# gcorso/disco-diffdock

Measured on AMD Instinct MI355X. Metric: complexes/sec, 20-step 40-sample inference, higher is better.
Workload: dtype f32

## Files before the change

disco_diffdock_amd/_lib.py:

```python
import ctypes as C
import os

_HERE = os.path.dirname(os.path.abspath(__file__))
LIB_PATH = os.environ.get('DDK_LIB') or os.path.join(_HERE, 'libddk.so')


class ddk_config(C.Structure):
    _fields_ = [('ns', C.c_int32), ('nv', C.c_int32), ('num_conv_layers', C.c_int32),
                ('sigma_embed_dim', C.c_int32), ('distance_embed_dim', C.c_int32), ('cross_distance_embed_dim', C.c_int32),
                ('lig_max_radius', C.c_float), ('rec_max_radius', C.c_float), ('cross_max_distance', C.c_float),
                ('center_max_distance', C.c_float), ('dynamic_max_cross', C.c_int32), ('embedding_scale', C.c_float),
                ('scale_by_sigma', C.c_int32), ('no_torsion', C.c_int32), ('batch_norm', C.c_int32),
                ('latent_dim', C.c_int32), ('latent_vocab', C.c_int32), ('latent_droprate', C.c_float),
                ('lm_embedding_dim', C.c_int32),
                ('tr_sigma_min', C.c_float), ('tr_sigma_max', C.c_float), ('rot_sigma_min', C.c_float),
                ('rot_sigma_max', C.c_float), ('tor_sigma_min', C.c_float), ('tor_sigma_max', C.c_float),
                ('device', C.c_int32), ('all_atoms', C.c_int32), ('num_confidence_outputs', C.c_int32),
                ('confidence_no_batchnorm', C.c_int32), ('conv_kernel', C.c_int32), ('deterministic', C.c_int32), ('confidence_mode', C.c_int32)]


class ddk_complex_desc(C.Structure):
    _fields_ = [('n_lig', C.c_int32), ('n_rec', C.c_int32), ('n_bond_edges', C.c_int32), ('n_rot', C.c_int32),
                ('n_rec_edges', C.c_int32), ('rec_feat_dim', C.c_int32),
                ('lig_x', C.c_void_p), ('bond_index', C.c_void_p), ('bond_attr', C.c_void_p), ('edge_mask', C.c_void_p),
                ('mask_rotate', C.c_void_p), ('rec_x', C.c_void_p), ('rec_pos', C.c_void_p), ('rec_edge_index', C.c_void_p)]


class ddk_atoms_desc(C.Structure):
    _fields_ = [('n_atom', C.c_int32), ('n_atom_edges', C.c_int32), ('atom_x', C.c_void_p), ('atom_pos', C.c_void_p),
                ('atom_edge_index', C.c_void_p), ('atom_rec_index', C.c_void_p)]


class ddk_trajectory(C.Structure):
    _fields_ = [('pos', C.c_void_p), ('scores', C.c_void_p), ('perturb', C.c_void_p), ('edge_counts', C.c_void_p)]


class ddk_perturbation(C.Structure):
    _fields_ = [('tr_update', C.c_void_p), ('rot_update', C.c_void_p), ('tor_update', C.c_void_p),
                ('tr_score', C.c_void_p), ('rot_score', C.c_void_p), ('tor_score', C.c_void_p)]


class ddk_match_options(C.Structure):
    _fields_ = [('popsize', C.c_int32), ('maxiter', C.c_int32), ('tol', C.c_float), ('polish_iters', C.c_int32), ('n_islands', C.c_int32),
                ('seed', C.c_uint64), ('stream_id', C.c_uint64)]


_lib = None

SYMBOLS = ['ddk_create', 'ddk_destroy', 'ddk_last_error', 'ddk_version', 'ddk_load_weights', 'ddk_finalize_weights',
           'ddk_set_score_norm_tables', 'ddk_tp_forward', 'ddk_tp_backward', 'ddk_rtp_forward', 'ddk_rtp_backward', 'ddk_rtp_backward_workspace', 'ddk_rconv_forward', 'ddk_rconv_backward', 'ddk_rconv_workspace', 'ddk_rhid_forward', 'ddk_rhid_backward', 'ddk_rhid_workspace', 'ddk_hconv_forward', 'ddk_hconv_backward', 'ddk_hconv_workspace', 'ddk_eemb_forward', 'ddk_eemb_backward', 'ddk_eemb_workspace', 'ddk_eemb_latent_forward', 'ddk_eemb_latent_backward', 'ddk_eemb_latent_workspace', 'ddk_gumbel_softmax_batch', 'ddk_gumbel_softmax_batch_backward', 'ddk_gumbel_pick_samples', 'ddk_rng_latent_keep', 'ddk_node_cross_entropy_batch', 'ddk_node_cross_entropy_batch_backward', 'ddk_rng_decoding_index', 'ddk_seg_sum', 'ddk_conv_forward', 'ddk_complex_create', 'ddk_complex_destroy',
           'ddk_score_forward', 'ddk_se3_update', 'ddk_sample', 'ddk_last_graph_stats', 'ddk_last_node_features',
           'ddk_profile_enable', 'ddk_profile_read', 'ddk_profile_read_forwards', 'ddk_set_latents', 'ddk_set_guidance',
           'ddk_set_keep_receptor_features', 'ddk_randomize_position', 'ddk_complex_set_atoms',
           'ddk_confidence_forward', 'ddk_score_confidence', 'ddk_pose_metrics', 'ddk_build_graph', 'ddk_set_receptive_field_pruning', 'ddk_ar_logits', 'ddk_ar_decode', 'ddk_confidence_status',
           'ddk_sample_trajectory', 'ddk_pose_pairwise_rmsd', 'ddk_pose_cluster',
           'ddk_ligand_automorphisms_workspace', 'ddk_ligand_automorphisms',
           'ddk_receptor_knn_graph_workspace', 'ddk_receptor_knn_graph', 'ddk_radius_graph_workspace', 'ddk_radius_graph',
           'ddk_ligand_transformation_mask_workspace', 'ddk_ligand_transformation_mask',
           'ddk_rng_noise', 'ddk_rng_initial', 'ddk_rng_uniform',
           'ddk_so3_rows', 'ddk_torus_score', 'ddk_rng_perturbation', 'ddk_score_matching_loss',
           'ddk_conformer_match_workspace', 'ddk_conformer_rmsd', 'ddk_conformer_match',
           'ddk_rng_perturbation_batch', 'ddk_rng_forward_times', 'ddk_modify_conformer_batch', 'ddk_randomize_position_batch', 'ddk_score_matching_loss_batch',
           'ddk_score_matching_loss_batch_backward']

DEBUG_SYMBOLS = ['ddk_debug_export', 'ddk_debug_read_edges', 'ddk_debug_conf_counts', 'ddk_debug_conf_table', 'ddk_debug_conf_nodes', 'ddk_debug_conf_edges', 'ddk_debug_kabsch', 'ddk_debug_axis_angle', 'ddk_debug_set_layer0_dedup', 'ddk_debug_read_patch', 'ddk_debug_split3', 'ddk_debug_conv_trace', 'ddk_debug_pool_stats', 'ddk_debug_set_conv_workgroups', 'ddk_debug_set_alloc_limit', 'ddk_debug_cross_mirror']


def lib():
    global _lib
    if _lib is not None:
        return _lib
    if not os.path.exists(LIB_PATH):
        raise RuntimeError(f'{LIB_PATH} not found: build the HIP extension first (python -m disco_diffdock_amd.build). '
                           'disco_diffdock_amd has no CPU fallback.')
    import torch
    L = C.CDLL(LIB_PATH)
    missing = [s for s in SYMBOLS + DEBUG_SYMBOLS if not hasattr(L, s)]
    if missing:
        raise RuntimeError(f'{LIB_PATH} does not export {", ".join(missing)}: it is stale, build the HIP extension again '
                           '(python -m disco_diffdock_amd.build). disco_diffdock_amd has no CPU fallback.')
    vp, i32, i64, f32 = C.c_void_p, C.c_int32, C.c_int64, C.c_float
    L.ddk_create.argtypes = [C.POINTER(ddk_config), C.POINTER(vp)]
    L.ddk_destroy.argtypes = [vp]
    L.ddk_destroy.restype = None
    L.ddk_last_error.argtypes = [vp]
    L.ddk_last_error.restype = C.c_char_p
    L.ddk_version.restype = C.c_char_p
    L.ddk_load_weights.argtypes = [vp, C.c_char_p, vp, C.POINTER(i64), i32]
    L.ddk_finalize_weights.argtypes = [vp]
    L.ddk_set_score_norm_tables.argtypes = [vp, vp, i32, vp, i32]
    L.ddk_tp_forward.argtypes = [vp, i32, vp, vp, vp, i64, vp, vp]
    L.ddk_tp_backward.argtypes = [vp, i32, vp, vp, vp, vp, i64, vp, vp, vp, vp]
    L.ddk_rtp_forward.argtypes = [vp, i32, vp, vp, vp, C.POINTER(i64), i32, vp, vp, i64, vp, vp]
    L.ddk_rtp_backward.argtypes = [vp, i32, vp, vp, vp, C.POINTER(i64), i32, vp, vp, vp, i64, vp, vp, vp, vp, vp, vp, vp]
    L.ddk_rtp_backward_workspace.argtypes = [i32, i64, i32]
    L.ddk_rtp_backward_workspace.restype = i64
    L.ddk_rconv_forward.argtypes = [vp, i32, vp, i64, i64, vp, vp, vp, vp, vp, vp, C.POINTER(i64), i32, vp, vp, i64, vp, vp, vp]
    L.ddk_rconv_backward.argtypes = [vp, i32, vp, i64, i64, vp, vp, vp, vp, vp, vp, vp, vp, C.POINTER(i64), i32, vp, vp, vp, i64, vp, vp, vp, vp, vp, vp, vp]
    L.ddk_rconv_workspace.argtypes = [i32, i64, i32, i64, i64, i32]
    L.ddk_rconv_workspace.restype = i64
    L.ddk_rhid_forward.argtypes = [vp, vp, i64, vp, vp, vp, C.POINTER(i64), i32, vp, vp, f32, C.c_uint64, i64, vp, vp]
    L.ddk_rhid_backward.argtypes = [vp, vp, i64, vp, vp, vp, vp, vp, vp, vp, vp, C.POINTER(i64), i32, vp, vp, f32, i64, vp, vp, vp, vp, vp, vp]
    L.ddk_rhid_workspace.argtypes = [i64, i32, i64]
    L.ddk_rhid_workspace.restype = i64
    L.ddk_hconv_forward.argtypes = [vp, i32, vp, i64, i64, vp, vp, vp, vp, vp, vp, vp, vp, i64, vp, vp, vp]
    L.ddk_hconv_backward.argtypes = [vp, i32, vp, i64, i64, vp, vp, vp, vp, vp, vp, vp, vp, vp, vp, vp, i64, vp, vp, vp, vp, vp, vp]
    L.ddk_hconv_workspace.argtypes = [i32, i64, i64, i64, i32]
    L.ddk_hconv_workspace.restype = i64
    eemb = [vp, vp, i64, vp, i64, vp, vp, vp, i32, vp, i64, vp, f32, f32, i32, vp, vp, vp, vp, f32, C.c_uint64]
    L.ddk_eemb_forward.argtypes = eemb + [i64, vp, vp, vp]
    L.ddk_eemb_backward.argtypes = eemb + [vp, i64, vp, vp, vp, vp, vp, vp]
    L.ddk_eemb_workspace.argtypes = [i64, i32]
    L.ddk_eemb_workspace.restype = i64
    latent = [vp, vp, i32, i32, vp, vp]
    L.ddk_eemb_latent_forward.argtypes = eemb + latent + [i64, vp, vp, vp]
    L.ddk_eemb_latent_backward.argtypes = eemb + latent + [vp, vp, vp, vp, vp, i64, vp, vp, vp, vp, vp, vp, vp, vp, vp]
    L.ddk_eemb_latent_workspace.argtypes = [i64, i32, i32]
    L.ddk_eemb_latent_workspace.restype = i64
    gumbel = [vp, i32, i32, vp, i64, vp, i64, vp, vp, f32]
    L.ddk_gumbel_softmax_batch.argtypes = gumbel + [C.c_uint64, vp, i32, i32, vp, vp, vp, vp, vp]
    L.ddk_gumbel_softmax_batch_backward.argtypes = gumbel + [vp, vp, vp, vp, vp]
    L.ddk_gumbel_pick_samples.argtypes = [vp, i32, i32, vp, i64, vp, i64, f32, C.c_uint64, C.c_uint64, i32, i32, vp, vp, vp, vp]
    L.ddk_rng_latent_keep.argtypes = [vp, C.c_uint64, i32, vp, i32, i32, f32, vp]
    node_ce = [vp, i32, i32, vp, i64, vp, i64, vp, vp, vp, vp, vp, i32]
    L.ddk_node_cross_entropy_batch.argtypes = node_ce + [vp, vp, vp, vp, vp]
    L.ddk_node_cross_entropy_batch_backward.argtypes = node_ce + [vp, vp, vp, vp, vp, vp]
    L.ddk_rng_decoding_index.argtypes = [vp, C.c_uint64, i32, vp, i32, i32, i32, vp]
    L.ddk_seg_sum.argtypes = [vp, vp, vp, vp, vp, i64, i32, vp]
    L.ddk_conv_forward.argtypes = [vp, i32, vp, i64, vp, vp, C.POINTER(i64), vp, vp, vp, vp]
    L.ddk_complex_create.argtypes = [vp, C.POINTER(ddk_complex_desc), i32, C.POINTER(vp)]
    L.ddk_complex_destroy.argtypes = [vp, vp]
    L.ddk_complex_destroy.restype = None
    L.ddk_score_forward.argtypes = [vp, vp, i32, vp, f32, f32, f32, vp, vp, vp, vp]
    L.ddk_se3_update.argtypes = [vp, vp, i32, vp, vp, vp, vp, vp, vp]
    L.ddk_randomize_position.argtypes = [vp, vp, i32, vp, vp, vp, vp, vp, vp]
    L.ddk_complex_set_atoms.argtypes = [vp, vp, vp, vp, vp, i32]
    L.ddk_confidence_forward.argtypes = [vp, vp, i32, vp, vp, vp]
    L.ddk_score_confidence.argtypes = [vp, vp, i32, vp, C.c_float, C.c_float, C.c_float, vp, vp]
    L.ddk_pose_metrics.argtypes = [vp, vp, i32, vp, vp, vp, vp, i32, vp, i32, vp, vp]
    L.ddk_pose_pairwise_rmsd.argtypes = [vp, i32, i32, vp, vp, vp, i32, vp, vp]
    L.ddk_pose_cluster.argtypes = [vp, i32, vp, vp, f32, vp, vp, vp, vp]
    L.ddk_ligand_automorphisms_workspace.argtypes = [i32, i32]
    L.ddk_ligand_automorphisms_workspace.restype = i64
    L.ddk_ligand_automorphisms.argtypes = [vp, i32, vp, vp, i32, vp, vp, i32, vp, vp, vp]
    for name in ('ddk_receptor_knn_graph_workspace', 'ddk_radius_graph_workspace', 'ddk_ligand_transformation_mask_workspace'):
        getattr(L, name).argtypes = [i32, i32]
        getattr(L, name).restype = i64
    L.ddk_receptor_knn_graph.argtypes = [vp, i32, vp, f32, i32, vp, i32, vp, vp, vp]
    L.ddk_radius_graph.argtypes = [vp, i32, vp, f32, i32, vp, i32, vp, vp, vp]
    L.ddk_ligand_transformation_mask.argtypes = [vp, i32, vp, i32, vp, vp, i32, vp, vp, vp]
    u64 = C.c_uint64
    L.ddk_rng_noise.argtypes = [vp, u64, u64, i32, i32, i32, i32, i32, i32, vp, vp, vp]
    L.ddk_rng_initial.argtypes = [vp, u64, u64, i32, i32, i32, f32, i32, vp, vp, vp, vp]
    L.ddk_rng_uniform.argtypes = [vp, u64, u64, i32, i32, i32, vp, vp]
    L.ddk_so3_rows.argtypes = [vp, i32, vp, vp, vp, vp, vp]
    L.ddk_torus_score.argtypes = [vp, i64, vp, i32, vp, vp]
    L.ddk_rng_perturbation.argtypes = [vp, u64, u64, i32, i32, i32, i32, f32, f32, i32, vp, vp, C.POINTER(ddk_perturbation), vp]
    L.ddk_score_matching_loss.argtypes = [vp, i32, i32, vp, vp, vp, vp, vp, vp, f32, f32, f32, vp, vp]
    L.ddk_rng_perturbation_batch.argtypes = [vp, u64, i32, vp, vp, vp, i32, i32, vp, vp, vp, vp, i32, vp, vp, C.POINTER(ddk_perturbation), vp]
    L.ddk_rng_forward_times.argtypes = [vp, u64, i32, vp, i32, i32, vp]
    L.ddk_modify_conformer_batch.argtypes = [vp, i32, i32, vp, vp, i32, vp, vp, vp, i32, vp, vp, vp, vp, vp, vp, vp]
    L.ddk_randomize_position_batch.argtypes = [vp, u64, i32, i32, vp, vp, i32, vp, vp, vp, i32, vp, vp, vp, f32, vp, vp, vp]
    L.ddk_score_matching_loss_batch.argtypes = [vp, i32, vp, i32, vp, vp, vp, vp, vp, vp, vp, vp, vp, vp, vp]
    L.ddk_score_matching_loss_batch_backward.argtypes = [vp, i32, vp, i32, vp, vp, vp, vp, vp, vp, vp, vp, vp, vp, vp, vp, vp, vp]
    L.ddk_conformer_match_workspace.argtypes = [i32, i32, i32, i32]
    L.ddk_conformer_match_workspace.restype = i64
    L.ddk_conformer_rmsd.argtypes = [vp, i32, vp, vp, vp, vp, vp, i32, i32, vp, vp, vp, vp]
    L.ddk_conformer_match.argtypes = [vp, i32, vp, vp, vp, vp, vp, i32, C.POINTER(ddk_match_options), vp, vp, vp, vp, vp, vp]
    L.ddk_sample.argtypes = [vp, vp, i32, i32, vp, vp, vp, vp, vp, vp]
    L.ddk_sample_trajectory.argtypes = [vp, vp, i32, i32, vp, vp, vp, vp, vp, C.POINTER(ddk_trajectory), vp]
    L.ddk_last_graph_stats.argtypes = [vp, vp, vp, vp]
    L.ddk_build_graph.argtypes = [vp, vp, C.c_int32, vp, C.c_float, vp, vp, C.c_int64, vp, vp]
    L.ddk_last_node_features.argtypes = [vp, vp, i32, vp, vp, vp]
    L.ddk_set_latents.argtypes = [vp, vp, vp, vp, f32]
    L.ddk_set_guidance.argtypes = [vp, vp, f32, f32, f32]
    L.ddk_set_keep_receptor_features.argtypes = [vp, vp, i32]
    L.ddk_profile_enable.argtypes = [vp, i32]
    L.ddk_set_receptive_field_pruning.argtypes = [vp, i32]
    L.ddk_ar_logits.argtypes = [vp, vp, i32, vp, vp]
    L.ddk_confidence_status.argtypes = [vp, vp, vp, vp]
    L.ddk_ar_decode.argtypes = [vp, vp, i32, vp, f32, vp, i32, i32, vp, vp, vp, vp]
    L.ddk_profile_read.argtypes = [vp, vp, i32]
    L.ddk_profile_read_forwards.argtypes = [vp, vp, i32]
    L.ddk_debug_export.argtypes = [vp, C.c_char_p, vp, i64]
    L.ddk_debug_export.restype = i64
    _declare_debug(L)
    _lib = L
    return L


def _declare_debug(L):
    import ctypes as C
    L.ddk_debug_read_edges.argtypes = [C.c_void_p, C.c_void_p, C.c_int64, C.c_int64, C.c_void_p, C.c_void_p, C.c_void_p, C.c_void_p,
                                       C.c_void_p, C.c_int64]
    L.ddk_debug_cross_mirror.argtypes = [C.c_void_p, C.c_void_p]
    L.ddk_debug_kabsch.argtypes = [C.c_void_p, C.c_int32, C.c_int32, C.c_void_p, C.c_void_p, C.c_void_p, C.c_void_p, C.c_void_p]
    L.ddk_debug_axis_angle.argtypes = [C.c_void_p, C.c_int32, C.c_void_p, C.c_void_p, C.c_void_p]
    L.ddk_debug_set_layer0_dedup.argtypes = [C.c_void_p, C.c_int32]
    L.ddk_debug_read_patch.argtypes = [C.c_void_p, C.c_void_p, C.c_int32, C.c_void_p, C.c_void_p]
    L.ddk_debug_split3.argtypes = [C.c_void_p, C.c_void_p, C.c_int64, C.c_int32, C.c_void_p, C.c_void_p, C.c_void_p, C.c_void_p, C.c_void_p]
    L.ddk_debug_conv_trace.argtypes = [C.c_void_p, C.c_int32, C.c_void_p]
    L.ddk_debug_pool_stats.argtypes = [C.c_void_p, C.c_void_p]
    L.ddk_debug_set_conv_workgroups.argtypes = [C.c_void_p, C.c_int32]
    L.ddk_debug_set_alloc_limit.argtypes = [C.c_void_p, C.c_int64]
    L.ddk_debug_conf_counts.argtypes = [C.c_void_p, C.c_void_p, C.c_void_p]
    L.ddk_debug_conf_table.argtypes = [C.c_void_p, C.c_void_p, C.c_int32, C.c_void_p]
    L.ddk_debug_conf_nodes.argtypes = [C.c_void_p, C.c_void_p, C.c_void_p, C.c_void_p, C.c_int64]
    L.ddk_debug_conf_edges.argtypes = [C.c_void_p, C.c_void_p, C.c_int64, C.c_int64, C.c_void_p, C.c_void_p, C.c_void_p, C.c_void_p, C.c_void_p]
```

disco_diffdock_amd/csrc/conv_launch.hip:

```cpp
#include "k_conv_common.h"
#include "k_node.h"
#include "model.h"

namespace ddk {

__global__ void conv_setup_kernel(int32_t* tile_info, int g0, int g1, int g2, int g3, int g4) {
  if (threadIdx.x == 0 && blockIdx.x == 0) {
    const int go[5] = {g0, g1, g2, g3, g4};
    int ts = 0;
    tile_info[0] = 0;
    for (int g = 0; g < 4; ++g) {
      ts += (go[g + 1] - go[g] + 31) / 32;
      tile_info[g + 1] = ts;
    }
    for (int g = 0; g < 5; ++g) tile_info[5 + g] = go[g];
    tile_info[10] = 0;
  }
}

__global__ void conv_one_group_kernel(int32_t* gt, int n_groups, int k, int E) {
  const int g = threadIdx.x;
  if (g < n_groups) { gt[g] = 0; gt[n_groups + g] = g == k ? E : 0; }
}

// ... 80 lines not shown
                                const float* bn_scale, const float* bn_bias, int64_t n, int dout, int out_stride,
                                float* out, hipStream_t s, const float* sum_rr0, int64_t n_lig_total, int n_rec, int clear_sum,
                                float* zero_extra, int64_t n_extra, int n_slots, const uint8_t* rr0_mask) {
  int64_t tot = n * out_stride;
  if (zero_extra != nullptr && n_extra > tot) tot = n_extra;
  if (tot == 0) return hipSuccess;
  hipLaunchKernelGGL(node_finalize_kernel, dim3((unsigned)((tot + 255) / 256)), dim3(256), 0, s, sum, deg, x_in, bn_mean,
                     bn_scale, bn_bias, n, dout, out_stride, out, sum_rr0, n_lig_total, n_rec, clear_sum, zero_extra, n_extra, n_slots, rr0_mask);
  return hipGetLastError();
}

__global__ __launch_bounds__(256) void conv_det_fix_kernel(ConvKArgs A, int dout) {
  const int lane = threadIdx.x & 63;
  int tile = blockIdx.x * 4 + (threadIdx.x >> 6);
  int g = 0, gb = 0, ge = 0, bstart = 0;
  if (A.det_nr > 0) {
    const int blk = tile / CONV_WAVES;
    if (blk >= A.det_rng[A.det_nr]) return;
    const DetRange R_ = det_find(A.det_rng, A.det_nr, blk);
    g = R_.g; gb = R_.beg; ge = R_.end; bstart = R_.bstart;
    tile -= bstart * CONV_WAVES;
    if (gb + 32 * tile >= ge) return;
  } else {
    for (; g < A.n_active; ++g) {
      gb = A.gbeg[g]; ge = A.gend[g];
      const int nt = (ge - gb + 31) / 32;
      if (tile < nt) break;
      tile -= nt;
      bstart += (ge - gb + CONV_BLOCK_EDGES - 1) / CONV_BLOCK_EDGES;
    }
    if (g >= A.n_active) return;
  }
  auto prow_of = [&](int t, int which) { return A.part + ((size_t)((bstart + t / CONV_WAVES) * CONV_WAVES + t % CONV_WAVES) * 2 + which) * XW; };
  int e0 = gb + 32 * tile;
  int n = min(32, ge - e0);
  const int s_last = A.src[e0 + n - 1];
  if (!(e0 + n < ge && A.src[e0 + n] == s_last)) return;
  if (A.src[e0] == s_last && e0 > gb && A.src[e0 - 1] == s_last) return;
  float acc0 = 0.0f, acc1 = 0.0f;
  const float* prow = prow_of(tile, 1);
  if (lane < dout) acc0 = prow[lane];
  if (lane + 64 < dout) acc1 = prow[lane + 64];
  for (;;) {
    ++tile;
    e0 += 32;
    n = min(32, ge - e0);
    prow = prow_of(tile, 0);
    if (lane < dout) acc0 += prow[lane];
    if (lane + 64 < dout) acc1 += prow[lane + 64];
    if (!(A.src[e0 + n - 1] == s_last && e0 + n < ge && A.src[e0 + n] == s_last)) break;
  }
  float* row = (A.sum_g2 != nullptr && g == 2) ? A.sum_g2 + (size_t)(s_last - A.g2_node_off) * XW
                                               : A.sum + ((size_t)s_last * A.n_slots + ((A.slots >> (2 * g)) & 3)) * XW;
  if (lane < dout) row[lane] = acc0;
  if (lane + 64 < dout) row[lane + 64] = acc1;
}

static void conv_det_fix(const ConvKArgs& k, const ConvLaunch& a, int dout, hipStream_t s) {
  const int64_t tiles = a.edge_bound / 32 + 8 * CONV_MAX_GROUPS + (int64_t)CONV_WAVES * a.det_nr;
  hipLaunchKernelGGL(conv_det_fix_kernel, dim3((unsigned)((tiles + 3) / 4)), dim3(256), 0, s, k, dout);
}

enum ConvFamily { CONV_F32, CONV_X3, CONV_X2 };
static ConvTable conv_table(int family) { return family == CONV_F32 ? conv_f32_table() : family == CONV_X3 ? conv_x3_table() : conv_x2_table(); }

static hipError_t conv_select(const ConvLayerDev& L, const ConvLaunch& a, ConvFamily& family, ConvKey& key) {
  const bool f16 = L.w2x != nullptr && (a.mode == 0 || (a.mode == 1 && a.pre == nullptr));
  family = !f16 ? CONV_F32 : L.limbs == 2 ? CONV_X2 : CONV_X3;
  key.gather = a.gather != 0; key.split = a.gather && a.pre != nullptr; key.det = a.part != nullptr; key.trace = false; key.mode = a.mode == 1 ? 1 : 0;
  if (family == CONV_F32) {
    if (key.det && a.mode != 0) return hipErrorInvalidValue;
    if (key.mode == 1) key.split = false;
  } else {
    if (family == CONV_X2 && key.split && !(L.sender_in_gemm1 && L.w1sx != nullptr)) return hipErrorInvalidValue;
    if (key.mode == 1) {
      if (a.pre != nullptr || a.part != nullptr || a.trace != nullptr) return hipErrorInvalidValue;
    } else if (!key.det) {
      if (key.split && !L.epi_ok) return hipErrorInvalidValue;
      key.trace = a.trace != nullptr;
      if (key.trace && !key.split) return hipErrorInvalidValue;
    }
  }
  if (key.det && key.gather && !key.split) return hipErrorInvalidValue;
  return hipSuccess;
}

static ConvXArgs conv_args(const ConvLayerDev& L, const ConvLaunch& a, bool f16, bool trace) {
  ConvXArgs X = {};
  ConvKArgs& k = X.k;
  k.x = a.x; k.src = a.src; k.dst = a.dst; k.edge_attr = a.edge_attr; k.sh = a.sh; k.sum = a.sum;
  k.counter = a.counter;
  k.b1p = L.b1p[0]; k.n_tiles = L.n_tiles;
  k.n_cols = L.n_cols;
  for (int c = 0; c <= L.n_cols; ++c) k.col_start[c] = L.col_start[c];
  k.sum_g2 = a.sum_g2; k.g2_node_off = a.g2_node_off;
  k.n_groups = a.n_groups; k.n_active = a.n_active; k.n_slots = a.n_slots; k.slots = a.slots; k.wmap = a.wmap;
  if (a.gbeg) { k.gbeg = a.gbeg; k.gend = a.gend; }
  else { k.gbeg = a.tile_info + 5; k.gend = a.tile_info + 6; }
  k.pre = a.pre; k.part = a.part; k.det_rng = a.det_rng; k.det_nr = a.det_nr;
  if (f16) {
    k.w1x = L.w1x; k.w1sx = L.w1sx; k.w2x = L.w2x;
    for (int g = 0; g < CONV_MAX_GROUPS; ++g) { k.w1s[g] = L.w1s[g]; k.w1u[g] = 1.0f / L.w1s[g]; k.w2s[g] = L.w2s[g]; k.w2u[g] = 1.0f / L.w2s[g]; }
  } else {
    k.w1p = L.w1p[0]; k.w2r = L.w2r[0];
    for (int g = 0; g < CONV_MAX_GROUPS; ++g) { k.w1s[g] = 1.0f; k.w1u[g] = 1.0f; k.w2s[g] = 1.0f; k.w2u[g] = 1.0f; }
  }
  X.trace = trace ? a.trace : nullptr; X.trace_coarse = a.trace_coarse;
  return X;
}

hipError_t conv_prepare_device() {
  for (int family = CONV_F32; family <= CONV_X2; ++family) {
    const ConvTable t = conv_table(family);
    for (int i = 0; i < t.n; ++i) {
      const hipError_t e = hipFuncSetAttribute(t.v[i].fn, hipFuncAttributeMaxDynamicSharedMemorySize, (int)t.v[i].lds);
      if (e != hipSuccess) return e;
    }
  }
  return hipSuccess;
}

hipError_t launch_conv_fused(const ConvLayerDev& L, const ConvLaunch& a, int n_cu, hipStream_t s) {
  ConvFamily family;
  ConvKey key;
  hipError_t e = conv_select(L, a, family, key);
  if (e != hipSuccess) return e;
  const ConvTable t = conv_table(family);
  const ConvVariant* v = nullptr;
  for (int i = 0; i < t.n && v == nullptr; ++i) {
    const ConvKey& q = t.v[i].key;
    if (q.gather == key.gather && q.split == key.split && q.det == key.det && q.trace == key.trace && q.mode == key.mode) v = t.v + i;
  }
  if (v == nullptr) return hipErrorInvalidValue;
  ConvXArgs X = conv_args(L, a, family != CONV_F32, key.trace);
  void* args[] = {family == CONV_F32 ? static_cast<void*>(&X.k) : static_cast<void*>(&X)};
  (void)hipLaunchKernel(v->fn, dim3(n_cu), dim3(v->threads), args, v->lds, s);
  e = hipGetLastError();
  if (e != hipSuccess || !key.det) return e;
  conv_det_fix(X.k, a, L.dout, s);
  return hipGetLastError();
}

}
```

disco_diffdock_amd/csrc/ddk_internal.h:

```cpp
#pragma once
#include <hip/hip_runtime.h>
#include <stdint.h>

#include <map>
#include <string>
#include <vector>

#include "../../include/ddk.h"
#include "../../include/ddk_debug.h"

namespace ddk {

constexpr int NS = 24;
constexpr int NV = 6;
constexpr int XW = 2 * NS + 6 * NV;
constexpr int NE = 3 * NS;
constexpr int OFF_P = NS;
constexpr int OFF_Q = NS + 3 * NV;
constexpr int OFF_C = NS + 6 * NV;

constexpr int F_A = 0;
constexpr int F_C = NS;
constexpr int F_T1O = 2 * NS;
constexpr int F_T1E = F_T1O + 6 * NV;
// ... 89 lines not shown
  int W = 0;
  int din = 0, dout = 0;
  float* w1p[4] = {};
  float* b1p[4] = {};
  float* w2r[4] = {};
  uint8_t* w1x = nullptr;
  uint8_t* w1sx = nullptr;
  uint8_t* w2x = nullptr;
  float w1s[CONV_MAX_GROUPS] = {1, 1, 1, 1, 1, 1, 1, 1, 1}, w2s[CONV_MAX_GROUPS] = {1, 1, 1, 1, 1, 1, 1, 1, 1};
  int limbs = 2;
  bool sender_in_gemm1 = false;
  bool epi_ok = false;
  int n_cols = 0;
  int col_start[17] = {};
  float* wn = nullptr;
  float* bnp = nullptr;
  std::vector<float> h_wn, h_bnp;
  float* bn_mean = nullptr;
  float* bn_scale = nullptr;
  float* bn_bias = nullptr;
  std::vector<std::vector<float>> h_w1p, h_b1p, h_w2p, h_b2p;
  std::vector<float> h_bn_mean, h_bn_scale, h_bn_bias;
  int n_groups = 4;
  std::vector<TileDesc> h_tiles;
  std::vector<uint8_t> h_w1x, h_w2x, h_w1sx;
  int n_in[4] = {}, n_out[4] = {}, blk_off[4] = {};
  int in_mul[4] = {}, out_mul[4] = {};
};

constexpr int PRE_W = 4 * NE;
static inline int pre_pos(int o) {
  const int r32 = o < 64 ? o % 32 : o - 64, hh = (r32 >> 2) & 1;
  return o < 64 ? hh * 36 + (o / 32) * 16 + (r32 & 3) + 4 * (r32 >> 3) : hh * 36 + 32 + (r32 & 3);
}

struct HostTensor {
  std::vector<int64_t> shape;
  std::vector<float> data;
};

struct Workspace {
  int32_t* tile_info = nullptr;
  float* xpad = nullptr;
  float* sum = nullptr;
  int32_t* deg = nullptr;
  size_t xpad_cap = 0, sum_cap = 0, deg_cap = 0;
  float* gumbel_y = nullptr;
  size_t gumbel_y_cap = 0;
};

}

namespace ddk { constexpr int PROF_INTS = 8; }

struct ddk_ctx {
  ddk_config cfg;
  std::string err;
  bool finalized = false;
  bool host_only = false;
  int n_cu = 256;
  int max_rec = 0;
  std::map<std::string, ddk::HostTensor> weights;
  std::vector<ddk::ConvLayerDev> conv;
  ddk::ConvLayerDev head[2];
  std::vector<double> so3_table, torus_table;
  ddk::Workspace ws;
  std::vector<void*> dev_allocs;
  int64_t dev_bytes = 0, alloc_limit = 0, alloc_refusals = 0;
  std::map<void*, size_t> dev_sizes;
  void* model = nullptr;
  void* conf_model = nullptr;
  hipStream_t up_stream = nullptr;
  hipStream_t head_stream = nullptr;
  hipEvent_t ev_fork = nullptr, ev_join = nullptr;
  struct StageBuf { char* p = nullptr; size_t cap = 0; hipEvent_t done = nullptr; bool in_flight = false; };
  std::vector<StageBuf> stage_pool;
  struct PoolChunk { void* p = nullptr; size_t cap = 0; hipEvent_t free_after = nullptr; };
  std::vector<PoolChunk> chunk_pool;
  size_t chunk_pool_bytes = 0;
  int64_t pool_mallocs = 0, pool_reuses = 0, pool_frees = 0, pool_bytes_out = 0, pool_bytes_out_peak = 0;
  bool prof = false;
  bool prune = true;
  uint32_t* conv_trace = nullptr; int conv_trace_layer = -1; int conv_trace_coarse = 0;
  bool layer0_dedup = true;
  struct ProfRec { hipEvent_t a, b; int layer; int slot; int tab = 0; int64_t r01_skipped = 0; bool lig_only = false; };
  std::vector<ProfRec> prof_recs;
  int32_t* prof_edges = nullptr;
  int prof_slots = 0, prof_cap = 0;
};

namespace ddk {
int fail(ddk_ctx* ctx, int code, const std::string& msg);
int hip_fail(ddk_ctx* ctx, hipError_t e, const char* what);
hipError_t ctx_malloc(ddk_ctx* ctx, void** p, size_t bytes);
void ctx_free(ddk_ctx* ctx, void* p);
size_t pool_evict_idle(ddk_ctx* ctx, bool wait);
void* dev_alloc(ddk_ctx* ctx, size_t bytes);
float* dev_upload(ddk_ctx* ctx, const std::vector<float>& v);
int ensure(ddk_ctx* ctx, void** p, size_t* cap, size_t bytes);

struct ConvLaunch {
  const float* x;
  const int32_t* src;
  const int32_t* dst;
  const float* edge_attr;
  const float* sh;
  float* sum;
  const int32_t* tile_info;
  int32_t* counter;
  float* part = nullptr;
  int64_t edge_bound = 0;
  const int32_t* det_rng = nullptr;
  int det_nr = 0;
  const float* pre = nullptr;
  int gather;
  float* sum_g2 = nullptr;
  int g2_node_off = 0;
  int mode = 0;
  int n_groups = 4, n_active = 4, n_slots = 1;
  uint32_t slots = 0;
  uint64_t wmap = 0x876543210ull;
  const int32_t* gbeg = nullptr;
  const int32_t* gend = nullptr;
  uint32_t* trace = nullptr;
  int trace_coarse = 0;
};
hipError_t launch_conv_fused(const ConvLayerDev& L, const ConvLaunch& a, int n_cu, hipStream_t s);
hipError_t launch_split3_probe(const float* x, int64_t n, int group, float* hi, float* mid, float* lo, float* scale, hipStream_t s);
int build_conv_layer(ddk_ctx* ctx, int mode, int l, ConvLayerDev& L);
int build_head_layer(ddk_ctx* ctx, int mode, ConvLayerDev& L);
hipError_t conv_prepare_device();
hipError_t graph_prepare_device(int* max_rec);
hipError_t launch_conv_setup(int32_t* tile_info, const int64_t* group_offsets_host, hipStream_t s);
hipError_t launch_conv_one_group(int32_t* gt, int n_groups, int k, int64_t E, hipStream_t s);
hipError_t launch_pad_rows(const float* x, int64_t n, int din, float* xpad, hipStream_t s);
hipError_t launch_count_deg(const int32_t* src, int64_t E, int32_t* deg, hipStream_t s);
struct NodePreArgs {
  float* sum; const int32_t* deg; const float* x_in; const float* bn_mean; const float* bn_scale; const float* bn_bias;
  int dout; float* x_out; const float* sum_rr0; int n_lig_total, n_rec_total, n_rec; float* zero_extra; int64_t n_extra; int n_slots;
  const float* wn; const float* bnp; float* pre;
  int lig_roles, rec_roles;
  const uint8_t* rr0_mask = nullptr;
  const uint8_t* levels; int max_level;
};
struct NodeEmbedArgs;
hipError_t launch_node_finalize_pre(const NodePreArgs& a, bool finalize, hipStream_t s, const NodeEmbedArgs* embed = nullptr);
hipError_t launch_node_finalize(float* sum, const int32_t* deg, const float* x_in ,
                                const float* bn_mean, const float* bn_scale, const float* bn_bias, int64_t n, int dout,
                                int out_stride, float* out, hipStream_t s, const float* sum_rr0 = nullptr,
                                int64_t n_lig_total = 0, int n_rec = 1, int clear_sum = 0, float* zero_extra = nullptr,
                                int64_t n_extra = 0, int n_slots = 1, const uint8_t* rr0_mask = nullptr);
hipError_t launch_tp_forward(const ConvLayerDev& L, const float* x_dst, const float* sh, const float* w, int64_t E,
                             float* out, hipStream_t s);
hipError_t launch_tp_backward(const ConvLayerDev& L, const float* x_dst, const float* sh, const float* w, const float* grad_out, int64_t E,
                              float* grad_x, float* grad_sh, float* grad_w, hipStream_t s);
hipError_t launch_rtp_forward(const ConvLayerDev& L, const float* x_dst, const float* sh, const float* h, const int64_t* group_offsets, int n_groups,
                              const float* w2, const float* b2, float* out, hipStream_t s);
hipError_t launch_rtp_backward(const ConvLayerDev& L, const float* x_dst, const float* sh, const float* h, const int64_t* group_offsets, int n_groups,
                               const float* w2, const float* b2, const float* grad_out, float* grad_x, float* grad_sh, float* grad_h, float* grad_w2,
                               float* grad_b2, float* workspace, hipStream_t s);
int64_t rtp_backward_workspace(int32_t layer, int64_t E, int32_t n_groups);
__host__ __device__ inline int64_t rtp_slice_len(int64_t E) {
  const int64_t l = ((E + 239) / 240 + 63) / 64 * 64;
  return l > 512 ? l : 512;
}
struct EdgeGroupTable { int64_t off[5]; int n_groups; };
struct GroupUnit { int grp; int64_t begin, end; };

inline EdgeGroupTable group_table(const int64_t* group_offsets, int n_groups) {
  EdgeGroupTable t{};
  for (int q = 0; q <= n_groups; ++q) t.off[q] = group_offsets[q];
  t.n_groups = n_groups;
  return t;
}
inline EdgeGroupTable group_table(int64_t E) { return EdgeGroupTable{{0, E, 0, 0, 0}, 1}; }

__host__ __device__ __forceinline__ GroupUnit group_unit(const EdgeGroupTable& t, int64_t b, int64_t per) {
  GroupUnit u{-1, 0, 0};
#pragma unroll
  for (int q = 0; q < 4; ++q) {
    if (q < t.n_groups && u.grp < 0) {
      const int64_t nb = (t.off[q + 1] - t.off[q] + per - 1) / per;
      if (b < nb) { u.grp = q; u.begin = t.off[q] + b * per; u.end = u.begin + per < t.off[q + 1] ? u.begin + per : t.off[q + 1]; } else b -= nb;
    }
  }
  return u;
}
inline void group_units(const EdgeGroupTable& t, int grp, int64_t per, int64_t& first, int64_t& count) {
  first = 0; count = 0;
  for (int q = 0; q < 4; ++q) {
    if (q < t.n_groups) {
      const int64_t n = (t.off[q + 1] - t.off[q] + per - 1) / per;
      if (q < grp) first += n;
      if (q == grp) count = n;
    }
  }
}
inline int64_t group_unit_total(const EdgeGroupTable& t, int64_t per) {
  int64_t n = 0;
  for (int q = 0; q < t.n_groups; ++q) n += (t.off[q + 1] - t.off[q] + per - 1) / per;
// ... 72 lines not shown
```

disco_diffdock_amd/csrc/k_conv.hip:

```cpp
#include <stdlib.h>

#include "k_conv_common.h"

namespace ddk {

__device__ __forceinline__ void load_frags(float4 (&a)[9], f32x16& B, const float* w, const float* b) {
#pragma unroll
  for (int s4 = 0; s4 < 9; ++s4) a[s4] = ld4(w + s4 * 256);
#pragma unroll
  for (int j = 0; j < 4; ++j) {
    const float4 v = ld4(b + 4 * j);
    B[4 * j + 0] = v.x; B[4 * j + 1] = v.y; B[4 * j + 2] = v.z; B[4 * j + 3] = v.w;
  }
}

__device__ __forceinline__ f32x16 burst(const float4 (&a)[9], const float (&h)[36], const f32x16& C) {
  f32x16 D = MFMA(a[0].x, h[0], C);
  D = MFMA(a[0].y, h[1], D);
  D = MFMA(a[0].z, h[2], D);
  D = MFMA(a[0].w, h[3], D);
#pragma unroll
  for (int s4 = 1; s4 < 9; ++s4) {
    D = MFMA(a[s4].x, h[4 * s4 + 0], D);
    D = MFMA(a[s4].y, h[4 * s4 + 1], D);
    D = MFMA(a[s4].z, h[4 * s4 + 2], D);
    D = MFMA(a[s4].w, h[4 * s4 + 3], D);
  }
  return D;
}

__device__ __forceinline__ void lds_frags(float4 (&a)[9], f32x16& B, const float* stage, int lane, int hh) {
#pragma unroll
  for (int s4 = 0; s4 < 9; ++s4) a[s4] = ld4(stage + s4 * 256 + lane * 4);
#pragma unroll
  for (int j = 0; j < 4; ++j) {
    const float4 v = ld4(stage + 2304 + hh * 16 + 4 * j);
    B[4 * j + 0] = v.x; B[4 * j + 1] = v.y; B[4 * j + 2] = v.z; B[4 * j + 3] = v.w;
  }
}

template <bool GATHER, int MODE, bool SPLIT, bool DET>
__global__ __launch_bounds__(64 * ConvTraits<MODE>::WAVES) void conv_fused_kernel(ConvKArgs A) {
  static_assert(!SPLIT || (GATHER && MODE == 0), "the GEMM1 split exists for the score model's gather path");
  static_assert(!DET || MODE == 0, "the deterministic scatter exists for the score model");
  constexpr int WAVES = ConvTraits<MODE>::WAVES, FS = ConvTraits<MODE>::FS, BLOCK_EDGES = 32 * WAVES;
  extern __shared__ __attribute__((aligned(16))) float lds[];
  const int tid = threadIdx.x, lane = tid & 63, wave = tid >> 6;
  float* F = lds + wave * (32 * FS);
  float* ring = lds + WAVES * (32 * FS);
  int* blk_slot = reinterpret_cast<int*>(ring + 2 * W2_TILE_FLOATS);
  const int el = lane & 31;
  const int hh = lane >> 5;
  const bool g2_shared = A.sum_g2 != nullptr;
  int gb_v = 0, ge_v = 0;
  if (lane < A.n_active) {
    gb_v = A.gbeg[lane];
    ge_v = A.gend[lane];
  }
  const int nb_v = (ge_v - gb_v + BLOCK_EDGES - 1) / BLOCK_EDGES;
  int pend_v = nb_v;
#pragma unroll
  for (int d = 1; d < 16; d *= 2) {
    const int t = __shfl_up(pend_v, d, 64);
    if (lane >= d) pend_v += t;
  }
  const int pbeg_v = pend_v - nb_v;
  int bs4 = __builtin_amdgcn_readlane(pend_v, 15);
  if constexpr (DET) {
    if (A.det_nr > 0) bs4 = A.det_rng[A.det_nr];
  }
  float* Fr = F + el * FS;
  const float inv_s3 = 0.57735026918962576451f, inv_s2 = 0.70710678118654752440f;
  const int n_tiles = A.n_tiles;
  constexpr int REC4 = W2_TILE_FLOATS / 4;
  const bool second = tid < REC4 - 64 * WAVES;

  const int nwg = gridDim.x;
  const int full = bs4 >= nwg ? (bs4 / nwg) * nwg : 0;
  const int rest = bs4 - full;
  int split = 1;
  if (rest > 0) {
    float best = 1e30f;
    for (int sp = 1; sp <= A.n_cols; ++sp) {
      const float cost = (float)((rest * sp + nwg - 1) / nwg) / (float)sp * (1.0f + 0.05f * (float)(sp - 1));
      if (cost < best - 1e-6f) { best = cost; split = sp; }
    }
  }
  const int n_units = full + rest * split;

  int unit = blockIdx.x;
  for (;;) {
    if (unit >= n_units) break;
    int unit_next = 0;
    if (tid == 0) unit_next = nwg + atomicAdd(A.counter, 1);
    int blk = unit, t_begin = 0, t_end = n_tiles;
    if (unit >= full) {
      const int r = unit - full, c = r % split;
      blk = full + r / split;
      t_begin = A.col_start[(c * A.n_cols) / split];
      t_end = A.col_start[((c + 1) * A.n_cols) / split];
    }
    int g = __popcll(__ballot(lane < 16 && blk >= pend_v));
    int gbeg = __builtin_amdgcn_readlane(gb_v, g), gend = __builtin_amdgcn_readlane(ge_v, g);
    int bstart = __builtin_amdgcn_readlane(pbeg_v, g);
    if constexpr (DET) {
      if (A.det_nr > 0) {
        const DetRange R_ = det_find(A.det_rng, A.det_nr, blk);
        g = R_.g; gbeg = R_.beg; gend = R_.end; bstart = R_.bstart;
      }
    }
    const int e0 = gbeg + BLOCK_EDGES * (blk - bstart) + 32 * wave;
    const int nvalid = min(32, gend - e0);
    const bool valid = el < nvalid;
    const int e = nvalid > 0 ? e0 + min(el, nvalid - 1) : gend - 1;
    const int sn = A.src[e], dn = A.dst[e];

    const int gw = (int)((A.wmap >> (4 * g)) & 15);
    const float* wrec = A.w2r + (size_t)gw * n_tiles * W2_TILE_FLOATS;
    {
      const float* wr0 = wrec + (size_t)t_begin * W2_TILE_FLOATS;
      const float* wr1 = wrec + (size_t)min(t_begin + 1, t_end - 1) * W2_TILE_FLOATS;
      const float4 r0 = ld4(wr0 + 4 * tid), r1 = ld4(wr1 + 4 * tid);
      *reinterpret_cast<float4*>(ring + 4 * tid) = r0;
      *reinterpret_cast<float4*>(ring + W2_TILE_FLOATS + 4 * tid) = r1;
      if (second) {
        const int q = 4 * (tid + 64 * WAVES);
        const float4 r2 = ld4(wr0 + q), r3 = ld4(wr1 + q);
        *reinterpret_cast<float4*>(ring + q) = r2;
        *reinterpret_cast<float4*>(ring + W2_TILE_FLOATS + q) = r3;
      }
    }

    const SegCtl seg = make_segctl(sn, el, nvalid, valid);

    float h[36];
    if constexpr (SPLIT) {
      float bin[12];
      {
        const float* pe = A.edge_attr + (size_t)e * NS + 12 * hh;
#pragma unroll
        for (int j = 0; j < 3; ++j) {
          const float4 a = ld4(pe + 4 * j);
          bin[4 * j + 0] = a.x; bin[4 * j + 1] = a.y; bin[4 * j + 2] = a.z; bin[4 * j + 3] = a.w;
        }
      }
      const float* ps = A.pre + ((size_t)sn * 4 + (gw & 1)) * NE + 36 * hh;
      const float* pd = A.pre + ((size_t)dn * 4 + 2 + (gw >> 1)) * NE + 36 * hh;
      const float* w1 = A.w1p + (size_t)gw * (3 * 9 * 64 * 4);
#pragma unroll
      for (int T = 0; T < 3; ++T) {
        f32x16 acc;
#pragma unroll
        for (int j = 0; j < 4; ++j) {
          if (T < 2 || j == 0) {
            const float4 u = ld4(ps + 16 * T + 4 * j), w = ld4(pd + 16 * T + 4 * j);
            acc[4 * j + 0] = u.x + w.x; acc[4 * j + 1] = u.y + w.y; acc[4 * j + 2] = u.z + w.z; acc[4 * j + 3] = u.w + w.w;
          } else {
            acc[4 * j + 0] = 0.0f; acc[4 * j + 1] = 0.0f; acc[4 * j + 2] = 0.0f; acc[4 * j + 3] = 0.0f;
          }
        }
        const float* wp = w1 + ((size_t)T * 9 * 64 + lane) * 4;
#pragma unroll
        for (int s4 = 0; s4 < 3; ++s4) {
          const float4 a = ld4(wp + s4 * 64 * 4);
          acc = MFMA(a.x, bin[4 * s4 + 0], acc);
          acc = MFMA(a.y, bin[4 * s4 + 1], acc);
          acc = MFMA(a.z, bin[4 * s4 + 2], acc);
          acc = MFMA(a.w, bin[4 * s4 + 3], acc);
        }
        if (T < 2) {
#pragma unroll
          for (int r = 0; r < 16; ++r) h[16 * T + r] = fmaxf(acc[r], 0.0f);
        } else {
#pragma unroll
          for (int r = 0; r < 4; ++r) h[32 + r] = fmaxf(acc[r], 0.0f);
        }
      }
    } else {
    float bin[36];
    {
      const float *pe, *pxs, *pxd;
      if (GATHER) {
        pe = A.edge_attr + (size_t)e * NS + 12 * hh;
        pxs = A.x + (size_t)sn * XW + 12 * hh;
        pxd = A.x + (size_t)dn * XW + 12 * hh;
      } else {
        pe = A.edge_attr + (size_t)e * NE + 12 * hh;
        pxs = pe + NS;
        pxd = pe + 2 * NS;
      }
#pragma unroll
      for (int j = 0; j < 3; ++j) {
        const float4 a = ld4(pe + 4 * j), b = ld4(pxs + 4 * j), c = ld4(pxd + 4 * j);
        bin[4 * j + 0] = a.x; bin[4 * j + 1] = a.y; bin[4 * j + 2] = a.z; bin[4 * j + 3] = a.w;
        bin[12 + 4 * j + 0] = b.x; bin[12 + 4 * j + 1] = b.y; bin[12 + 4 * j + 2] = b.z; bin[12 + 4 * j + 3] = b.w;
        bin[24 + 4 * j + 0] = c.x; bin[24 + 4 * j + 1] = c.y; bin[24 + 4 * j + 2] = c.z; bin[24 + 4 * j + 3] = c.w;
      }
    }
    {
      const float* w1 = A.w1p + (size_t)gw * (3 * 9 * 64 * 4);
      const float* b1 = A.b1p + (size_t)gw * (3 * 2 * 16);
#pragma unroll
      for (int T = 0; T < 3; ++T) {
        f32x16 acc;
        const float* bp = b1 + (T * 2 + hh) * 16;
#pragma unroll
        for (int j = 0; j < 4; ++j) {
          const float4 b = ld4(bp + 4 * j);
          acc[4 * j + 0] = b.x; acc[4 * j + 1] = b.y; acc[4 * j + 2] = b.z; acc[4 * j + 3] = b.w;
        }
        const float* wp = w1 + ((size_t)T * 9 * 64 + lane) * 4;
#pragma unroll
        for (int s4 = 0; s4 < 9; ++s4) {
          const float4 a = ld4(wp + s4 * 64 * 4);
          acc = MFMA(a.x, bin[4 * s4 + 0], acc);
          acc = MFMA(a.y, bin[4 * s4 + 1], acc);
          acc = MFMA(a.z, bin[4 * s4 + 2], acc);
          acc = MFMA(a.w, bin[4 * s4 + 3], acc);
        }
        if (T < 2) {
#pragma unroll
          for (int r = 0; r < 16; ++r) h[16 * T + r] = fmaxf(acc[r], 0.0f);
        } else {
#pragma unroll
          for (int r = 0; r < 4; ++r) h[32 + r] = fmaxf(acc[r], 0.0f);
        }
      }
    }
    }

    const float4 shv = ld4(A.sh + (size_t)e * 4);
    const float s0 = shv.x, vx = shv.y, vy = shv.z, vz = shv.w;
    {
      const float* xr = A.x + (size_t)dn * XW;
      const int o_main_src = hh ? OFF_C : 0, o_main_dst = hh ? F_C : F_A;
      const int o_vec_src = hh ? OFF_Q : OFF_P;
      const int o_vs = hh ? F_T1E : F_T1O, o_vc = hh ? F_T1O : F_T1E, r0 = hh ? NV : 0;
#pragma unroll
      for (int j = 0; j < NS / 4; ++j) *reinterpret_cast<float4*>(Fr + o_main_dst + 4 * j) = ld4(xr + o_main_src + 4 * j);
      float pv[3 * NV];
#pragma unroll
      for (int j = 0; j < 3 * NV / 2; ++j) {
        const float2 t = ld2(xr + o_vec_src + 2 * j);
        pv[2 * j] = t.x; pv[2 * j + 1] = t.y;
      }
#pragma unroll
      for (int m = 0; m < NV; ++m) {
        const float px = pv[3 * m], py = pv[3 * m + 1], pz = pv[3 * m + 2];
        Fr[F_PQ + (m < 4 ? 4 * hh + m : 8 + 2 * hh + (m - 4))] = (px * vx + py * vy + pz * vz) * inv_s3;
        const int r = r0 + m;
        float* Ps = Fr + o_vs + 12 * (r >> 2) + (r & 3);
        float* Pc = Fr + o_vc + 12 * (r >> 2) + (r & 3);
        Ps[0] = px * s0;
        Ps[4] = py * s0;
        Ps[8] = pz * s0;
        Pc[0] = (py * vz - pz * vy) * inv_s2;
        Pc[4] = (pz * vx - px * vz) * inv_s2;
        Pc[8] = (px * vy - py * vx) * inv_s2;
        if (MODE == 1) {
          const float dv = (px * vx + py * vy + pz * vz) * (1.0f / 3.0f);
          const float n3 = (vx * vx + vy * vy + vz * vz) * (1.0f / 9.0f);
          float* P2 = Fr + (hh ? F_T2E : F_T2O) + 12 * (m >> 2) + (m & 3);
          P2[0] = dv * vx - px * n3;
          P2[4] = dv * vy - py * n3;
          P2[8] = dv * vz - pz * n3;
        }
      }
      if (MODE == 1) {
        float* P2 = Fr + (hh ? F_T2E : F_T2O) + 12;
        P2[2] = 0.0f; P2[3] = 0.0f; P2[6] = 0.0f; P2[7] = 0.0f; P2[10] = 0.0f; P2[11] = 0.0f;
      }
    }
    __syncthreads();

    float* node_row = (g2_shared && g == 2) ? A.sum_g2 + (size_t)(sn - A.g2_node_off) * XW
                                            : A.sum + ((size_t)sn * A.n_slots + ((A.slots >> (2 * g)) & 3)) * XW;
    if constexpr (DET) {
      if (nvalid > 0) {
        const int sn0 = __shfl(sn, 0, 32), snl = __shfl(sn, nvalid - 1, 32);
        const bool first_cont = e0 > gbeg && A.src[e0 - 1] == sn0;
        const bool last_cont = e0 + nvalid < gend && A.src[e0 + nvalid] == snl;
        float* prow = A.part + ((size_t)(blk * WAVES + wave) * 2) * XW;
        if (sn == sn0 && first_cont) node_row = prow;
        else if (sn == snl && last_cont) node_row = prow + XW;
      }
    }
    f32x2 accA[4], accV[4][3];
#pragma unroll
    for (int rq = 0; rq < 4; ++rq) { accA[rq] = 0.0f; accV[rq][0] = 0.0f; accV[rq][1] = 0.0f; accV[rq][2] = 0.0f; }
    float4 a0[9], a1[9];
    f32x16 B0, B1;
    lds_frags(a0, B0, ring, lane, hh);
    int2 tqv = *reinterpret_cast<const int2*>(ring + 2336);
    __syncthreads();
    TileQ tq;
    tq.w0 = __builtin_amdgcn_readfirstlane(tqv.x); tq.chan0 = __builtin_amdgcn_readfirstlane(tqv.y);
#define PSUM(p) ((p).x + (p).y)
#define DDK_EPILOGUE tile_epilogue(w0 & 3, D, f0, f1, f2, accA, accV);
#define DDK_FLUSH_COND ((w0 >> 2) & 3)
#define DDK_TILE_BARRIER __syncthreads();
#define DDK_TILE(T, AC, BC, AN, BN)                                                                            \
    {                                                                                                          \
      const int w0 = tq.w0, chan0 = tq.chan0;                                                                  \
      const int t2 = min((T) + 2, t_end - 1);                                                                  \
      const float* rec2 = wrec + (size_t)t2 * W2_TILE_FLOATS;                                                  \
      const float4 st0 = ld4(rec2 + 4 * tid);                                                                  \
      float4 st1 = make_float4(0.f, 0.f, 0.f, 0.f);        \
      if (second) st1 = ld4(rec2 + 4 * (tid + 64 * WAVES));                                                    \
      const float* Fp = Fr + (w0 >> 16);                                                                       \
      const f32x4 f0 = ldv4(Fp), f1 = ldv4(Fp + 4), f2 = ldv4(Fp + 8);                                        \
      lds_frags(AN, BN, ring + (((T) + 1 - t_begin) & 1) * W2_TILE_FLOATS, lane, hh);                                    \
      tqv = *reinterpret_cast<const int2*>(ring + (((T) + 1 - t_begin) & 1) * W2_TILE_FLOATS + 2336);          \
      __builtin_amdgcn_sched_barrier(0);                                                                       \
      const f32x16 D = burst(AC, h, BC);                                                                       \
// ... 67 lines not shown
```

disco_diffdock_amd/csrc/k_conv_common.h:

```cpp
#pragma once
#include "ddk_internal.h"

namespace ddk {

typedef float f32x16 __attribute__((ext_vector_type(16)));

struct ConvKArgs {
  const float* x;
  const int32_t* src;
  const int32_t* dst;
  const float* edge_attr;
  const float* sh;
  const float* pre;
  float* sum;
  int32_t* counter;
  const float* w1p;
  const float* b1p;
  const float* w2r;
  const uint8_t* w1x;
  const uint8_t* w1sx;
  const uint8_t* w2x;
  float w1s[CONV_MAX_GROUPS], w1u[CONV_MAX_GROUPS], w2s[CONV_MAX_GROUPS], w2u[CONV_MAX_GROUPS];
  int n_tiles;
  int n_cols;
  int col_start[17];
  float* part;
  float* sum_g2;
  int g2_node_off;
  int n_groups, n_active, n_slots;
  uint32_t slots;
  uint64_t wmap;
  const int32_t* gbeg;
  const int32_t* gend;
  const int32_t* det_rng = nullptr;
  int det_nr = 0;
};
struct DetRange { int beg, end, g, bstart; };
__device__ __forceinline__ DetRange det_find(const int32_t* rng, int nr, int blk) {
  int lo = 0, hi = nr;
  while (hi - lo > 1) {
    const int mid = (lo + hi) >> 1;
    if (rng[mid] <= blk) lo = mid; else hi = mid;
  }
  DetRange r;
  r.bstart = rng[lo]; r.beg = rng[nr + 1 + lo]; r.end = rng[2 * nr + 1 + lo]; r.g = rng[3 * nr + 1 + lo];
  return r;
}

struct ConvXArgs {
  ConvKArgs k;
  uint32_t* trace;
  int trace_coarse;
};
struct ConvKey { bool gather, split, det, trace; int mode; };
struct ConvVariant { ConvKey key; const void* fn; int threads; size_t lds; };
struct ConvTable { const ConvVariant* v; int n; };
ConvTable conv_f32_table();
ConvTable conv_x3_table();
ConvTable conv_x2_table();

bool conv_epilogue_shapes_ok(const std::vector<TileDesc>& tiles);

__device__ __forceinline__ float4 ld4(const float* p) { return *reinterpret_cast<const float4*>(p); }
__device__ __forceinline__ float2 ld2(const float* p) { return *reinterpret_cast<const float2*>(p); }

#define MFMA(a, b, c) __builtin_amdgcn_mfma_f32_32x32x2f32((a), (b), (c), 0, 0, 0)

struct TileQ { int w0, chan0; };

typedef float f32x2 __attribute__((ext_vector_type(2)));
typedef float f32x4 __attribute__((ext_vector_type(4)));
__device__ __forceinline__ f32x4 ldv4(const float* p) { return *reinterpret_cast<const f32x4*>(p); }
#define D_LO(D, rq) (f32x2{(D)[4 * (rq)], (D)[4 * (rq) + 1]})
#define D_HI(D, rq) (f32x2{(D)[4 * (rq) + 2], (D)[4 * (rq) + 3]})
#define V_LO(f) __builtin_shufflevector(f, f, 0, 1)
#define V_HI(f) __builtin_shufflevector(f, f, 2, 3)

__device__ __forceinline__ void tile_epilogue(int kind, const f32x16& D, f32x4 f0, f32x4 f1, f32x4 f2, f32x2 (&accA)[4],
                                              f32x2 (&accV)[4][3]) {
  f32x2 fhi = V_HI(f0);
  if (kind == T_RTS) fhi = 0.0f;
  if (kind == T_RA) {
#pragma unroll
    for (int rq = 0; rq < 4; ++rq) accA[rq] = __builtin_elementwise_fma(D_HI(D, rq), fhi, __builtin_elementwise_fma(D_LO(D, rq), V_LO(f0), accA[rq]));
  }
  if (kind != T_RA) {
#pragma unroll
    for (int rq = 0; rq < 4; ++rq) accV[rq][0] = __builtin_elementwise_fma(D_HI(D, rq), fhi, __builtin_elementwise_fma(D_LO(D, rq), V_LO(f0), accV[rq][0]));
  }
  if (kind == T_TV) {
#pragma unroll
    for (int rq = 0; rq < 4; ++rq) {
      accV[rq][1] = __builtin_elementwise_fma(D_HI(D, rq), V_HI(f1), __builtin_elementwise_fma(D_LO(D, rq), V_LO(f1), accV[rq][1]));
      accV[rq][2] = __builtin_elementwise_fma(D_HI(D, rq), V_HI(f2), __builtin_elementwise_fma(D_LO(D, rq), V_LO(f2), accV[rq][2]));
    }
  }
}

struct SegCtl { bool m1, m2, m4, m8, m16, tail, valid; };

__device__ __forceinline__ SegCtl make_segctl(int sn, int el, int nvalid, bool valid) {
  SegCtl c;
  const int prev = __shfl_up(sn, 1, 32);
  const int next = __shfl_down(sn, 1, 32);
  const int r = (el == 0) || (prev != sn);
  c.tail = valid && ((el == nvalid - 1) || (next != sn));
  c.valid = valid;
  const int rl = el & 15;
  int f = r | (rl == 0);
  int g = r;
  int fu, gu;
  fu = __shfl_up(f, 1, 32); gu = __shfl_up(g, 1, 32); c.m1 = !f; if (rl >= 1) { f |= fu; g |= gu; }
  fu = __shfl_up(f, 2, 32); gu = __shfl_up(g, 2, 32); c.m2 = !f; if (rl >= 2) { f |= fu; g |= gu; }
  fu = __shfl_up(f, 4, 32); gu = __shfl_up(g, 4, 32); c.m4 = !f; if (rl >= 4) { f |= fu; g |= gu; }
  fu = __shfl_up(f, 8, 32); gu = __shfl_up(g, 8, 32); c.m8 = !f; if (rl >= 8) { f |= fu; g |= gu; }
  c.m16 = (el >= 16) && !g;
  return c;
}

// ... 56 lines not shown
```

disco_diffdock_amd/csrc/k_conv_x.hip:

```cpp
#include <stdlib.h>

#include "k_conv_common.h"

#ifdef X3_TWO_LIMBS
#define conv_x3_kernel conv_x2_kernel
#define conv_x3_table conv_x2_table
#include "k_conv_x_epi2_gen.inc"
#define X3_TILE_BYTES W2X2_TILE_BYTES
#define X3_BIAS_OFF W2X2_BIAS_OFF
#define X3_DESC_OFF W2X2_DESC_OFF
#define X3_W1_TILE_BYTES W1X2_TILE_BYTES
#define X3_LDS_BYTES CONV_X2_LDS_BYTES
#define X3_W1L_BYTES W1L_BYTES
#define X3_TWO true
#define X3_SUM(r) D0[r]
#define X3_TAIL3(a_lh, a_hm) (void)(a_lh); D0 = MFMA16(a_hm, HT.mh, D0); D0 = MFMA16(a_hm, HT.hm, D0);
#define X3_STEP(MF, ah, am, al, bh, bm, bl)   \
  (void)(al);                                 \
  D0 = MF(ah, bm, D0);                        \
  D0 = MF(am, bh, D0);                        \
  D0 = MF(ah, bh, D0);
#define X3_FRAG(f, off) f.h = *reinterpret_cast<const f16x8*>(ringl + (off)); f.m = *reinterpret_cast<const f16x8*>(ringl + W2X_LIMB_BYTES + (off));
#define X3_TAIL_LO(SO) th
#define X3_TRIO(mask) { __builtin_amdgcn_sched_group_barrier(0x008, 1, 0); __builtin_amdgcn_sched_group_barrier(mask, 1, 0); __builtin_amdgcn_sched_group_barrier(0x100, 1, 0); }
// ... 156 lines not shown
    a23[2] = fmaf(f2.z, d2, fmaf(f2.w, d3, a23[2]));
  }
}
__device__ __forceinline__ void tv_rows_l2(const f32x16& D, f32x4 f0, f32x4 f1, f32x4 f2, float (&accY)[3][3]) {
#pragma unroll
  for (int rq = 0; rq < TVQ; ++rq) {
    const float d0 = D[4 * rq], d1 = D[4 * rq + 1], d2 = D[4 * rq + 2], d3 = D[4 * rq + 3];
    accY[rq][0] = fmaf(f0.x, d0, fmaf(f0.y, d1, fmaf(f0.z, d2, fmaf(f0.w, d3, accY[rq][0]))));
    accY[rq][1] = fmaf(f1.x, d0, fmaf(f1.y, d1, fmaf(f1.z, d2, fmaf(f1.w, d3, accY[rq][1]))));
    accY[rq][2] = fmaf(f2.x, d0, fmaf(f2.y, d1, fmaf(f2.z, d2, fmaf(f2.w, d3, accY[rq][2]))));
  }
}
template <int MODE>
__device__ __forceinline__ void tile_epilogue_s(int w0, const f32x16& D, const float* Fp, f32x4 f0, float (&accA)[4], float (&accV)[4][3],
                                                float (&accX)[4][3], float (&accY)[3][3]) {
  const int kind = w0 & 3;
  if (MODE == 1 && kind == T_TV && (w0 & X_TILE_L2)) {
    const f32x4 f1 = ldv4(Fp + 4), f2 = ldv4(Fp + 8);
    tv_rows_l2(D, f0, f1, f2, accY);
  } else if (kind == T_TV) {
    const f32x4 f1 = ldv4(Fp + 4), f2 = ldv4(Fp + 8);
    switch ((w0 >> 14) & 3) {
      case 0: tv_rows<false, false>(D, f0, f1, f2, accV, accX); break;
      case 1: tv_rows<true, false>(D, f0, f1, f2, accV, accX); break;
      case 2: tv_rows<false, true>(D, f0, f1, f2, accV, accX); break;
      default: tv_rows<true, true>(D, f0, f1, f2, accV, accX); break;
    }
  } else if (kind == T_RA) {
#pragma unroll
    for (int rq = 0; rq < 4; ++rq)
      accA[rq] = fmaf(f0.x, D[4 * rq], fmaf(f0.y, D[4 * rq + 1], fmaf(f0.z, D[4 * rq + 2], fmaf(f0.w, D[4 * rq + 3], accA[rq]))));
  } else if (kind == T_RT) {
#pragma unroll
    for (int rq = 0; rq < 4; ++rq)
      accV[rq][0] = fmaf(f0.x, D[4 * rq], fmaf(f0.y, D[4 * rq + 1], fmaf(f0.z, D[4 * rq + 2], fmaf(f0.w, D[4 * rq + 3], accV[rq][0]))));
  } else {
#pragma unroll
    for (int rq = 0; rq < 4; ++rq) accV[rq][0] = fmaf(f0.x, D[4 * rq], fmaf(f0.y, D[4 * rq + 1], accV[rq][0]));
  }
}

constexpr float UNIT_PROLOGUE_TILES = 6.5f;
template <bool GATHER, bool SPLIT, bool DET, bool TRACE = false, int MODE = 0>
__global__ __launch_bounds__(64 * CONV_WAVES) void conv_x3_kernel(ConvXArgs AX) {
  static_assert(!SPLIT || GATHER, "the GEMM1 split exists for the gather path");
  static_assert(MODE == 0 || (!SPLIT && !DET && !TRACE), "the confidence model runs the plain paths");
  int trace_n = 0;
  auto stamp = [&](int phase) {
    if constexpr (TRACE) {
      if (AX.trace_coarse == 1 && phase < 4) return;
      if (blockIdx.x == 0 && (threadIdx.x & 63) == 0 && trace_n < CONV_TRACE_TILES)
        AX.trace[((threadIdx.x >> 6) * CONV_TRACE_TILES + trace_n) * 8 + phase] = (uint32_t)__builtin_amdgcn_s_memtime();
      if (phase == 3) ++trace_n;
    }
  };
  bool first_tile = true;
  auto stamp_epi = [&](int slot) {
    if constexpr (TRACE) {
      if (AX.trace_coarse != 2 || first_tile) return;
      if (blockIdx.x == 0 && (threadIdx.x & 63) == 0 && trace_n < CONV_TRACE_TILES)
        AX.trace[((threadIdx.x >> 6) * CONV_TRACE_TILES + trace_n) * 8 + slot] = (uint32_t)__builtin_amdgcn_s_memtime();
    }
  };
  auto stamp_unit = [&](int slot, int value) {
    if constexpr (TRACE) {
      if (AX.trace_coarse != 1) return;
      if (blockIdx.x == 0 && (threadIdx.x & 63) == 0 && trace_n < CONV_TRACE_TILES)
        AX.trace[((threadIdx.x >> 6) * CONV_TRACE_TILES + trace_n) * 8 + slot] = slot == 1 ? (uint32_t)value : (uint32_t)__builtin_amdgcn_s_memtime();
      if (slot == 2) ++trace_n;
    }
  };
  const ConvKArgs& A = AX.k;
  constexpr int WAVES = CONV_WAVES, FS = FX_STRIDE, BLOCK_EDGES = 32 * WAVES;
  extern __shared__ __attribute__((aligned(16))) float lds[];
  const int tid = threadIdx.x, lane = tid & 63, wave = tid >> 6;
  float* F = lds + wave * (32 * FS);
  char* ring = reinterpret_cast<char*>(lds + WAVES * (32 * FS));
  char* w1l = ring + W2X_STAGES * X3_TILE_BYTES;
  int* blk_slot = reinterpret_cast<int*>(w1l + X3_W1L_BYTES);
  (void)w1l;
  const int el = lane & 31;
  const int hh = lane >> 5;
  const bool g2_shared = A.sum_g2 != nullptr;
  int gb_v = 0, ge_v = 0;
  if (lane < A.n_active) {
    gb_v = A.gbeg[lane];
    ge_v = A.gend[lane];
  }
  const int nb_v = (ge_v - gb_v + BLOCK_EDGES - 1) / BLOCK_EDGES;
  int pend_v = nb_v;
#pragma unroll
  for (int d = 1; d < 16; d *= 2) {
    const int t = __shfl_up(pend_v, d, 64);
    if (lane >= d) pend_v += t;
  }
  const int pbeg_v = pend_v - nb_v;
  int bs4 = __builtin_amdgcn_readlane(pend_v, 15);
  if constexpr (DET) {
    if (A.det_nr > 0) bs4 = A.det_rng[A.det_nr];
  }
  float* Fr = F + el * FS;
  const float inv_s3 = 0.57735026918962576451f, inv_s2 = 0.70710678118654752440f;
  const int n_tiles = A.n_tiles;
  constexpr int REC16 = X3_TILE_BYTES / 16;
  const int grp = wave >> 2;
  const uint32_t fo0 = 16u * tid, fo1 = 16u * min(tid + 64 * WAVES, REC16 - 1);
  const bool has1 = !X3_TWO || tid + 64 * WAVES < REC16;
  const unsigned long long c1_mask = __ballot(has1);
  const bool has1_s = !X3_TWO || c1_mask != 0;
  (void)has1; (void)has1_s; (void)c1_mask;
  int gw_lds = -1;
  (void)gw_lds;
  constexpr bool ASM_EPI = GATHER && SPLIT && !DET && MODE == 0;
  const unsigned ring0_u = (unsigned)(WAVES * 32 * FS * 4), ringb_u = ring0_u + 64u * hh, ringw0_u = ring0_u + fo0, ringw1_u = ring0_u + fo1;
  const unsigned fra_u = (unsigned)((wave * 32 + el) * FS * 4), hh4_u = 4u * hh, hh12_u = 12u * hh;
  int t0_, t1_, t2_, sel_, pk0_, pk1_, pk2_;
  unsigned long long sv_;
  (void)ringb_u; (void)ringw0_u; (void)ringw1_u; (void)fra_u; (void)hh4_u; (void)hh12_u;

  const int nwg = gridDim.x;
  const int full = bs4 >= nwg ? (bs4 / nwg) * nwg : 0;
  const int rest = bs4 - full;
  int split = 1;
  if (rest > 0) {
    float best = 1e30f;
    for (int sp = 1; sp <= A.n_cols; ++sp) {
      const float cost = (float)((rest * sp + nwg - 1) / nwg) * ((float)n_tiles / (float)sp + UNIT_PROLOGUE_TILES);
      if (cost < best - 1e-6f) { best = cost; split = sp; }
    }
  }
  const int n_units = full + rest * split;

  int unit = blockIdx.x;
  for (;;) {
    if (unit >= n_units) break;
    stamp(4);
    first_tile = true;
    int unit_next = 0;
    if (tid == 0) unit_next = nwg + atomicAdd(A.counter, 1);
    int blk = unit, t_begin = 0, t_end = n_tiles;
    if (unit >= full) {
      const int r = unit - full, c = r % split;
      blk = full + r / split;
      t_begin = A.col_start[(c * A.n_cols) / split];
      t_end = A.col_start[((c + 1) * A.n_cols) / split];
    }
    int g = __popcll(__ballot(lane < 16 && blk >= pend_v));
    int gbeg = __builtin_amdgcn_readlane(gb_v, g), gend = __builtin_amdgcn_readlane(ge_v, g);
    int bstart = __builtin_amdgcn_readlane(pbeg_v, g);
    if constexpr (DET) {
      if (A.det_nr > 0) {
        const DetRange R_ = det_find(A.det_rng, A.det_nr, blk);
        g = R_.g; gbeg = R_.beg; gend = R_.end; bstart = R_.bstart;
      }
    }
    const int e0 = gbeg + BLOCK_EDGES * (blk - bstart) + 32 * wave;
    const int nvalid = min(32, gend - e0);
    const bool valid = el < nvalid;
    const int e = nvalid > 0 ? e0 + min(el, nvalid - 1) : gend - 1;
    const int sn = A.src[e], dn = A.dst[e];

    const int gw = (int)((A.wmap >> (4 * g)) & 15);
    const char* wrec = reinterpret_cast<const char*>(A.w2x) + (size_t)gw * n_tiles * X3_TILE_BYTES;
    {
      const char* wr0 = wrec + (size_t)t_begin * X3_TILE_BYTES;
      const char* wr1 = wrec + (size_t)min(t_begin + 1, t_end - 1) * X3_TILE_BYTES;
      const char* wr2 = wrec + (size_t)min(t_begin + 2, t_end - 1) * X3_TILE_BYTES;
      const float4 r0 = *reinterpret_cast<const float4*>(wr0 + fo0);
      const float4 r2 = *reinterpret_cast<const float4*>(wr1 + fo0);
      const float4 r4 = *reinterpret_cast<const float4*>(wr2 + fo0);
      if (has1_s) { if (has1) {
        const float4 r1 = *reinterpret_cast<const float4*>(wr0 + fo1);
        const float4 r3 = *reinterpret_cast<const float4*>(wr1 + fo1);
        const float4 r5 = *reinterpret_cast<const float4*>(wr2 + fo1);
        *reinterpret_cast<float4*>(ring + fo1) = r1;
        *reinterpret_cast<float4*>(ring + X3_TILE_BYTES + fo1) = r3;
        *reinterpret_cast<float4*>(ring + 2 * X3_TILE_BYTES + fo1) = r5;
      } }
      *reinterpret_cast<float4*>(ring + fo0) = r0;
      *reinterpret_cast<float4*>(ring + X3_TILE_BYTES + fo0) = r2;
      *reinterpret_cast<float4*>(ring + 2 * X3_TILE_BYTES + fo0) = r4;
    }
#ifdef X3_TWO_LIMBS
    if constexpr (SPLIT) {
      static_assert(W1L_BYTES / 16 == 2 * 64 * CONV_WAVES + 128, "the copy below moves 1152 chunks");
      const int gw_s = __builtin_amdgcn_readfirstlane(gw);
      if (gw_s != gw_lds) {
        const char* wsrc = reinterpret_cast<const char*>(A.w1sx) + (size_t)gw_s * W1L_BYTES;
        const float4 c0 = *reinterpret_cast<const float4*>(wsrc + 16 * tid);
        const float4 c1 = *reinterpret_cast<const float4*>(wsrc + 16 * (tid + 64 * WAVES));
        if (wave < 2) {
          const float4 c2 = *reinterpret_cast<const float4*>(wsrc + 16 * (tid + 128 * WAVES));
          *reinterpret_cast<float4*>(w1l + 16 * (tid + 128 * WAVES)) = c2;
        }
        *reinterpret_cast<float4*>(w1l + 16 * tid) = c0;
        *reinterpret_cast<float4*>(w1l + 16 * (tid + 64 * WAVES)) = c1;
        gw_lds = gw_s;
        lds_barrier();
      }
    }
#endif

    const SegF seg = make_segf(make_segctl(sn, el, nvalid, valid));
    stamp(5);

    constexpr bool SENDK = SPLIT && X3_TWO;
    float4 shv;
    float4 mainv[NS / 4];
    float2 pv2[3 * NV / 2];
    const float* xr = A.x + (size_t)dn * XW;
    if constexpr (!SENDK) {
      shv = ld4(A.sh + (size_t)e * 4);
#pragma unroll
      for (int j = 0; j < NS / 4; ++j) mainv[j] = ld4(xr + (hh ? OFF_C : 0) + 4 * j);
#pragma unroll
      for (int j = 0; j < 3 * NV / 2; ++j) pv2[j] = ld2(xr + (hh ? OFF_Q : OFF_P) + 2 * j);
    }

    Limbs H;
    TailB HT;
    float osc, bsc2;
    {
      float h[36];
      const char* w1 = reinterpret_cast<const char*>(A.w1x) + (size_t)gw * 3 * X3_W1_TILE_BYTES;
      (void)w1;
      if constexpr (SPLIT) {
#ifdef X3_TWO_LIMBS
        float4 psv[9];
        {
          const float* ps = A.pre + ((size_t)sn * 4 + (gw & 1)) * NE + 36 * hh;
#pragma unroll
          for (int j = 0; j < 9; ++j) psv[j] = ld4(ps + 4 * j);
        }
        float bin[24];
        {
          const float* pe = A.edge_attr + (size_t)e * NS + 12 * hh;
#pragma unroll
          for (int j = 0; j < 3; ++j) {
            const float4 a = ld4(pe + 4 * j);
            bin[4 * j + 0] = a.x; bin[4 * j + 1] = a.y; bin[4 * j + 2] = a.z; bin[4 * j + 3] = a.w;
          }
#pragma unroll
          for (int j = 0; j < 3; ++j) mainv[j] = ld4(xr + 12 * hh + 4 * j);
        }
        shv = ld4(A.sh + (size_t)e * 4);
#pragma unroll
        for (int j = 0; j < 3; ++j) mainv[3 + j] = ld4(xr + OFF_C + 12 * hh + 4 * j);
#pragma unroll
        for (int j = 0; j < 3 * NV / 2; ++j) pv2[j] = ld2(xr + (hh ? OFF_Q : OFF_P) + 2 * j);
#pragma unroll
        for (int j = 0; j < 3; ++j) { bin[12 + 4 * j + 0] = mainv[j].x; bin[12 + 4 * j + 1] = mainv[j].y; bin[12 + 4 * j + 2] = mainv[j].z; bin[12 + 4 * j + 3] = mainv[j].w; }
        float m1 = 0.0f;
#pragma unroll
        for (int j = 0; j < 24; ++j) m1 = fmaxf(m1, fabsf(bin[j]));
        m1 = fmaxf(m1, __shfl_xor(m1, 32));
        float inv1;
        const float s1 = range_scale(m1, inv1);
        f16x8 bh[3], bm[3];
#pragma unroll
        for (int k = 0; k < 3; ++k)
#pragma unroll
          for (int i = 0; i < 8; ++i) { const Limb3 q = split3(bin[8 * k + i] * s1); bh[k][i] = q.h; bm[k][i] = q.m; }
        const float bsc = s1 * A.w1s[gw], usc = inv1 * A.w1u[gw];
#pragma unroll
        for (int T = 0; T < 3; ++T) {
          f32x16 D0;
#pragma unroll
          for (int j = 0; j < 4; ++j) {
            if (T < 2 || j == 0) {
              const float4 u = psv[4 * T + j];
              D0[4 * j + 0] = u.x * bsc; D0[4 * j + 1] = u.y * bsc; D0[4 * j + 2] = u.z * bsc; D0[4 * j + 3] = u.w * bsc;
            } else {
              D0[4 * j + 0] = 0.0f; D0[4 * j + 1] = 0.0f; D0[4 * j + 2] = 0.0f; D0[4 * j + 3] = 0.0f;
            }
          }
          const char* wt = w1l + T * (2 * W1L_LIMB_BYTES) + lane * 16;
#pragma unroll
          for (int k = 0; k < 3; ++k) {
            const f16x8 ah = *reinterpret_cast<const f16x8*>(wt + k * 1024), am = *reinterpret_cast<const f16x8*>(wt + W1L_LIMB_BYTES + k * 1024);
            X3_STEP(MFMA16, ah, am, ah, bh[k], bm[k], bh[k])
          }
          const int nr = T < 2 ? 16 : 4;
#pragma unroll
          for (int r = 0; r < 16; ++r)
            if (r < nr) h[16 * T + r] = fmaxf(D0[r], 0.0f) * usc;
        }
#else
        float4 psv[9], pdv[9];
        {
          const float* ps = A.pre + ((size_t)sn * 4 + (gw & 1)) * NE + 36 * hh;
          const float* pd = A.pre + ((size_t)dn * 4 + 2 + (gw >> 1)) * NE + 36 * hh;
#pragma unroll
          for (int j = 0; j < 9; ++j) { psv[j] = ld4(ps + 4 * j); pdv[j] = ld4(pd + 4 * j); }
        }
        float bin[12];
        {
          const float* pe = A.edge_attr + (size_t)e * NS + 12 * hh;
#pragma unroll
          for (int j = 0; j < 3; ++j) {
            const float4 a = ld4(pe + 4 * j);
            bin[4 * j + 0] = a.x; bin[4 * j + 1] = a.y; bin[4 * j + 2] = a.z; bin[4 * j + 3] = a.w;
          }
        }
        float m1 = 0.0f;
#pragma unroll
        for (int j = 0; j < 12; ++j) m1 = fmaxf(m1, fabsf(bin[j]));
        m1 = fmaxf(m1, __shfl_xor(m1, 32));
        float inv1;
        const float s1 = range_scale(m1, inv1);
        f16x8 b0h, b0m, b0l;
        f16x4 b1h, b1m, b1l;
#pragma unroll
        for (int i = 0; i < 8; ++i) { const Limb3 q = split3(bin[i] * s1); b0h[i] = q.h; b0m[i] = q.m; b0l[i] = q.l; }
#pragma unroll
        for (int i = 0; i < 4; ++i) { const Limb3 q = split3(bin[8 + i] * s1); b1h[i] = q.h; b1m[i] = q.m; b1l[i] = q.l; }
        const f16x8 b1_mh = __builtin_shufflevector(b1m, b1h, 0, 1, 2, 3, 4, 5, 6, 7), b1_hl = __builtin_shufflevector(b1h, b1l, 0, 1, 2, 3, 4, 5, 6, 7),
                    b1_hm = __builtin_shufflevector(b1h, b1m, 0, 1, 2, 3, 4, 5, 6, 7);
        const float bsc = s1 * A.w1s[gw], usc = inv1 * A.w1u[gw];
#pragma unroll
        for (int T = 0; T < 3; ++T) {
          f32x16 D0, D1;
#pragma unroll
          for (int j = 0; j < 4; ++j) {
            if (T < 2 || j == 0) {
              const float4 u = psv[4 * T + j], w = pdv[4 * T + j];
              D0[4 * j + 0] = (u.x + w.x) * bsc; D0[4 * j + 1] = (u.y + w.y) * bsc; D0[4 * j + 2] = (u.z + w.z) * bsc; D0[4 * j + 3] = (u.w + w.w) * bsc;
            } else {
              D0[4 * j + 0] = 0.0f; D0[4 * j + 1] = 0.0f; D0[4 * j + 2] = 0.0f; D0[4 * j + 3] = 0.0f;
            }
          }
#pragma unroll
          for (int r = 0; r < 16; ++r) D1[r] = 0.0f;
          const W1Split wf = w1_split(w1, T, lane);
          X3_STEP(MFMA16, wf.h, wf.m, wf.l, b0h, b0m, b0l)
          {
            const f16x4 ah = wf.th, am = wf.tm, al = wf.tl;
            const f16x8 a_hm = __builtin_shufflevector(ah, am, 0, 1, 2, 3, 4, 5, 6, 7), a_lh = __builtin_shufflevector(al, ah, 0, 1, 2, 3, 4, 5, 6, 7);
            D0 = MFMA16(a_hm, b1_mh, D0);
            D1 = MFMA16(a_lh, b1_hl, D1);
            D0 = MFMA16(a_hm, b1_hm, D0);
          }
          const int nr = T < 2 ? 16 : 4;
#pragma unroll
          for (int r = 0; r < 16; ++r)
            if (r < nr) h[16 * T + r] = fmaxf(X3_SUM(r), 0.0f) * usc;
        }
#endif
      } else {
        float bin[36];
        {
          const float *pe, *pxs, *pxd;
          if (GATHER) {
            pe = A.edge_attr + (size_t)e * NS + 12 * hh;
            pxs = A.x + (size_t)sn * XW + 12 * hh;
            pxd = A.x + (size_t)dn * XW + 12 * hh;
          } else {
            pe = A.edge_attr + (size_t)e * NE + 12 * hh;
            pxs = pe + NS;
            pxd = pe + 2 * NS;
          }
#pragma unroll
          for (int j = 0; j < 3; ++j) {
            const float4 a = ld4(pe + 4 * j), b = ld4(pxs + 4 * j), c = ld4(pxd + 4 * j);
            bin[4 * j + 0] = a.x; bin[4 * j + 1] = a.y; bin[4 * j + 2] = a.z; bin[4 * j + 3] = a.w;
            bin[12 + 4 * j + 0] = b.x; bin[12 + 4 * j + 1] = b.y; bin[12 + 4 * j + 2] = b.z; bin[12 + 4 * j + 3] = b.w;
            bin[24 + 4 * j + 0] = c.x; bin[24 + 4 * j + 1] = c.y; bin[24 + 4 * j + 2] = c.z; bin[24 + 4 * j + 3] = c.w;
          }
        }
        float m1 = 0.0f;
#pragma unroll
        for (int j = 0; j < 36; ++j) m1 = fmaxf(m1, fabsf(bin[j]));
        m1 = fmaxf(m1, __shfl_xor(m1, 32));
        float inv1;
        const float s1 = range_scale(m1, inv1);
        Limbs Bn;
        make_limbs(Bn, bin, s1);
        const float bsc = s1 * A.w1s[gw], usc = inv1 * A.w1u[gw];
        const float* b1 = A.b1p + (size_t)gw * (3 * 2 * 16);
#pragma unroll
        for (int T = 0; T < 3; ++T) {
          f32x16 D0, D1;
          const float* bp = b1 + (T * 2 + hh) * 16;
#pragma unroll
          for (int j = 0; j < 4; ++j) {
            const float4 b = ld4(bp + 4 * j);
            D0[4 * j + 0] = b.x * bsc; D0[4 * j + 1] = b.y * bsc; D0[4 * j + 2] = b.z * bsc; D0[4 * j + 3] = b.w * bsc;
          }
#pragma unroll
          for (int r = 0; r < 16; ++r) D1[r] = 0.0f;
          const char* wt = w1 + (size_t)T * X3_W1_TILE_BYTES;
#pragma unroll
          for (int s = 0; s < 4; ++s) {
            const f16x8 ah = *reinterpret_cast<const f16x8*>(wt + s * 1024 + lane * 16);
            const f16x8 am = *reinterpret_cast<const f16x8*>(wt + W2X_LIMB_BYTES + s * 1024 + lane * 16);
            const f16x8 al = w1_lo<f16x8>(wt + 2 * W2X_LIMB_BYTES + s * 1024 + lane * 16, ah);
            X3_STEP(MFMA16, ah, am, al, Bn.hi[s], Bn.mid[s], Bn.lo[s])
          }
          {
            const f16x4 ah = *reinterpret_cast<const f16x4*>(wt + 4096 + lane * 8);
            const f16x4 am = *reinterpret_cast<const f16x4*>(wt + W2X_LIMB_BYTES + 4096 + lane * 8);
            const f16x4 al = w1_lo<f16x4>(wt + 2 * W2X_LIMB_BYTES + 4096 + lane * 8, ah);
            X3_STEP(MFMA8, ah, am, al, Bn.thi, Bn.tmid, Bn.tlo)
          }
          const int nr = T < 2 ? 16 : 4;
#pragma unroll
          for (int r = 0; r < 16; ++r)
            if (r < nr) h[16 * T + r] = fmaxf(X3_SUM(r), 0.0f) * usc;
        }
      }
      float m2 = 0.0f;
#pragma unroll
      for (int j = 0; j < 36; ++j) m2 = fmaxf(m2, h[j]);
      m2 = fmaxf(m2, __shfl_xor(m2, 32));
      float inv2;
      const float s2 = range_scale(m2, inv2);
      stamp(6);
      make_limbs(H, h, s2);
      HT = make_tailb(H);
      bsc2 = s2 * A.w2s[gw];
      osc = inv2 * A.w2u[gw];
    }

    const float s0 = shv.x, vx = shv.y, vy = shv.z, vz = shv.w;
    {
      const int o_main_dst = hh ? FX_C : FX_A, r0 = hh ? NV : 0;
#pragma unroll
      for (int j = 0; j < NS / 4; ++j) {
        if constexpr (SENDK) *reinterpret_cast<float4*>(Fr + (j < 3 ? FX_A : FX_C - 12) + 12 * hh + 4 * j) = mainv[j];
        else *reinterpret_cast<float4*>(Fr + o_main_dst + 4 * j) = mainv[j];
      }
      float pv[3 * NV];
#pragma unroll
      for (int j = 0; j < 3 * NV / 2; ++j) { pv[2 * j] = pv2[j].x; pv[2 * j + 1] = pv2[j].y; }
#pragma unroll
      for (int m = 0; m < NV; ++m) {
        const float px = pv[3 * m], py = pv[3 * m + 1], pz = pv[3 * m + 2];
// ... 265 lines not shown
```

disco_diffdock_amd/csrc/k_graph.hip:

```cpp
#include <stdlib.h>
#include "model.h"
#include "k_node.h"

namespace ddk {


__device__ __forceinline__ bool cross_within(const float* lp, const float* rp, float c) {
#pragma clang fp contract(off)
  const float dx = rp[0] / c - lp[0] / c, dy = rp[1] / c - lp[1] / c, dz = rp[2] / c - lp[2] / c;
  return dx * dx + dy * dy + dz * dz < 1.0f;
}

__device__ __forceinline__ bool cross_within4(const float4 a, float rx, float ry, float rz) {
#pragma clang fp contract(off)
  const float dx = rx - a.x, dy = ry - a.y, dz = rz - a.z;
  return dx * dx + dy * dy + dz * dz < 1.0f;
}

__device__ __forceinline__ float dist2(const float* a, const float* b) {
#pragma clang fp contract(off)
  const float dx = a[0] - b[0], dy = a[1] - b[1], dz = a[2] - b[2];
  return dx * dx + dy * dy + dz * dz;
}

// ... 101 lines not shown
      b0 += l == 0 ? od : 0; b1 += l == 1 ? od : 0; b2 += l == 2 ? od : 0; b3 += l == 3 ? od : 0;
    }
  }
  if (tid < 4) { int t_ = 0; for (int w = 0; w < nw; ++w) t_ += tmp[w][tid]; tot[tid] = t_; }
  __syncthreads();
}

__global__ __launch_bounds__(GT) void graph_count_kernel(GraphArgs G) {
  extern __shared__ float smem[];
  float* lp = smem;
  float* rp = lp + MAX_LIG * 3;
  uint8_t* lvl = reinterpret_cast<uint8_t*>(rp + 3 * G.n_rec + G.n_rec);
  __shared__ unsigned adj[MAX_LIG][MAX_LIG / 32];
  __shared__ float4 lps[MAX_LIG];
  __shared__ int s_cnt[2], lvl_tmp[GT / 64][4], lvl_tot[4];
  const int b = blockIdx.x, tid = threadIdx.x;
  for (int i = tid; i < G.n_lig * 3; i += GT) {
    const float v = G.lig_pos[(size_t)b * G.n_lig * 3 + i];
    lp[i] = v;
    reinterpret_cast<float*>(lps)[4 * (i / 3) + i % 3] = v / G.cross_cutoff;
  }
  for (int i = tid; i < G.n_rec * 3; i += GT) rp[i] = G.rec_pos[i] / G.cross_cutoff;
  if (tid < 2) s_cnt[tid] = 0;
  __syncthreads();
  build_lig_adj(lp, G.n_lig, G.lig_r2, adj);
  __syncthreads();
  int c_ll = 0, c_lr = 0;
  for (int i = tid; i < G.n_lig; i += GT)
    for (int w = 0; w < MAX_LIG / 32; ++w) c_ll += __popc(adj[i][w]);
  for (int j = tid; j < G.n_rec; j += GT) {
    const float rx = rp[3 * j], ry = rp[3 * j + 1], rz = rp[3 * j + 2];
    int cnt = 0;
#pragma unroll 4
    for (int i = 0; i < G.n_lig; ++i) cnt += cross_within4(lps[i], rx, ry, rz) ? 1 : 0;
    c_lr += cnt;
    lvl[j] = (G.prune && cnt == 0) ? 3 : 0;
  }
#pragma unroll
  for (int d = 32; d > 0; d >>= 1) { c_ll += __shfl_down(c_ll, d, 64); c_lr += __shfl_down(c_lr, d, 64); }
  if ((tid & 63) == 0) { atomicAdd(&s_cnt[0], c_ll); atomicAdd(&s_cnt[1], c_lr); }
  __syncthreads();
  if (G.prune) propagate_levels(lvl, G);
  level_scan(lvl, G.rr_outdeg, G.n_rec, nullptr, lvl_tmp, lvl_tot);
  if (tid < 2) G.counts[CNT_STRIDE * b + tid] = s_cnt[tid];
  if (tid < 3) G.counts[CNT_STRIDE * b + 2 + tid] = lvl_tot[tid];
  for (int j = tid; j < G.n_rec; j += GT) G.levels[(size_t)b * G.n_rec + j] = lvl[j];
}

__device__ __forceinline__ void sample_prefix(const GraphArgs& G, int b, int* ex, int* tot) {
  const int lane = threadIdx.x & 63;
#pragma unroll
  for (int k = 0; k < 5; ++k) { tot[k] = 0; ex[k] = 0; }
  for (int b0 = 0; b0 < G.B; b0 += 64) {
    const int bb = b0 + lane;
    int v[5], inc[5];
#pragma unroll
    for (int k = 0; k < 5; ++k) v[k] = bb < G.B ? G.counts[CNT_STRIDE * bb + k] + (k == 0 ? G.M : 0) : 0;
#pragma unroll
    for (int k = 0; k < 5; ++k) {
      int x = v[k];
#pragma unroll
      for (int d = 1; d < 64; d *= 2) { const int t = __shfl_up(x, d, 64); if (lane >= d) x += t; }
      inc[k] = x;
    }
    if (b >= b0 && b < b0 + 64) {
#pragma unroll
      for (int k = 0; k < 5; ++k) ex[k] = tot[k] + __shfl(inc[k] - v[k], b - b0, 64);
    }
#pragma unroll
    for (int k = 0; k < 5; ++k) tot[k] += __shfl(inc[k], 63, 64);
  }
  ex[5] = b * G.E_rr - (ex[2] + ex[3] + ex[4]);
}

__device__ void write_group_tables(const GraphArgs& G, const int* tot) {
  const int ll = tot[0], lr = tot[1], ra = tot[2], rb = tot[3], rc = tot[4];
  int go[5];
  go[0] = 0; go[1] = ll; go[2] = ll + lr; go[3] = go[2] + G.B * G.E_rr; go[4] = go[3] + lr;
  const int seg[4] = {go[2], go[2] + ra, go[2] + ra + rb, go[2] + ra + rb + rc};
  const int n_shared = G.shared_rr ? G.E_rr : 0;
  int bs = 0;
  G.info[I_FB] = 0;
  for (int g = 0; g < 5; ++g) {
    bs += (g == 3 && G.cross_mirror) ? 0 : ((g < 4 ? go[g + 1] - go[g] : n_shared) + 255) / 256;
    G.info[I_FB + 1 + g] = bs;
  }
  for (int g = 0; g < 5; ++g) G.info[I_GO + g] = go[g];
  for (int k = 0; k < 8; ++k) G.info[I_CNT + k] = 0;
  for (int l = 0; l < 4; ++l) G.info[I_SEG + l] = seg[l];
  G.info[I_E] = go[4];
  G.info[I_OVF] = ((int64_t)go[4] + n_shared > G.edge_cap) ? 1 : 0;
  G.info[I_SHARED] = G.shared_rr ? go[4] : -1;
  G.info[I_HEAD] = 0; G.info[I_HEAD + 1] = G.B * G.n_lig; G.info[I_HEAD + 2] = G.B * G.n_lig; G.info[I_HEAD + 3] = G.B * G.n_lig;
  G.info[I_HEAD + 4] = 0; G.info[I_HEAD + 5] = 0;
  G.info[I_EXEC] = go[4];
  G.info[I_EXEC + 1] = go[2];
  G.info[I_EXEC + 7] = lr;
  for (int k = 0; k < N_TAB; ++k) {
    int32_t* tb = G.info + I_TAB + 8 * k;
    int tot = 0;
    for (int g = 0; g < 4; ++g) { tb[g] = go[g]; tb[4 + g] = go[g + 1]; }
    if (k == TAB_A) tb[4 + 2] = seg[1];
    if (k == TAB_B) tb[4 + 2] = seg[2];
    if (k == TAB_C) tb[4 + 2] = seg[3];
    if (k == TAB_SHARED) { tb[2] = go[4]; tb[4 + 2] = go[4] + n_shared; }
    for (int g = 0; g < 4; ++g) tot += tb[4 + g] - tb[g];
    if (k == TAB_SHARED && G.patch_off >= 0 && G.shared_rr) tot += G.info[I_PATCH];
    G.info[I_EXEC + 2 + k] = tot;
  }
  if (G.patch_off >= 0 && G.shared_rr) {
    const int np = G.info[I_PATCH];
    const int32_t* ts = G.info + I_TAB + 8 * TAB_SHARED;
    for (int g = 0; g < 4; ++g) { G.info[I_TABX + g] = ts[g]; G.info[I_TABX + 5 + g] = ts[4 + g]; }
    G.info[I_TABX + 4] = (int)G.patch_off; G.info[I_TABX + 9] = (int)G.patch_off + np;
    G.info[I_FBX] = bs + (np + 255) / 256;
  } else {
    G.info[I_FBX] = bs;
  }
}

__device__ __forceinline__ bool latent_nonzero(const float* lat, int64_t row, int ld) {
  bool nz = false;
  for (int j = 0; j < ld; ++j) nz |= lat[row * ld + j] != 0.0f;
  return nz;
}

__global__ __launch_bounds__(256) void disco_patch_count_kernel(PatchArgs A) {
  extern __shared__ unsigned char mk[];
  __shared__ int red[256];
  const int b = blockIdx.x, tid = threadIdx.x;
  for (int j = tid; j < A.n_rec; j += 256)
    mk[j] = b > 0 && (latent_nonzero(A.rec_latent, (int64_t)b * A.n_rec + j, A.latent_dim) || latent_nonzero(A.rec_latent, j, A.latent_dim));
  __syncthreads();
  int cnt = 0;
  for (int i = tid; i < A.n_rec; i += 256) {
    bool a = mk[i];
    const int k0 = A.rr_start[i], k1 = k0 + A.rr_outdeg[i];
    for (int k = k0; k < k1 && !a; ++k) a = mk[A.rr_dst[k]];
    A.rr_mask[(size_t)b * A.n_rec + i] = a;
    if (a) cnt += k1 - k0;
  }
  red[tid] = cnt;
  __syncthreads();
  for (int d = 128; d > 0; d >>= 1) { if (tid < d) red[tid] += red[tid + d]; __syncthreads(); }
  if (tid == 0) A.patch_cnt[b] = red[0];
}

__global__ void disco_patch_scan_kernel(PatchArgs A) {
  if (threadIdx.x != 0 || blockIdx.x != 0) return;
  int tot = 0;
  for (int b = 0; b < A.B; ++b) { const int c = A.patch_cnt[b]; A.patch_cnt[b] = tot; tot += c; }
  A.patch_cnt[A.B] = tot;
  A.info[I_PATCH] = tot;
}

__global__ __launch_bounds__(256) void disco_patch_fill_kernel(PatchArgs A) {
  extern __shared__ int pre_[];
  __shared__ int scan_tmp[16];
  const int b = blockIdx.x, tid = threadIdx.x;
  for (int i = tid; i < A.n_rec; i += 256) pre_[i] = A.rr_mask[(size_t)b * A.n_rec + i] ? A.rr_outdeg[i] : 0;
  __syncthreads();
  block_exclusive_scan(pre_, A.n_rec, scan_tmp);
  const int rec0 = A.B * A.n_lig + b * A.n_rec;
  const int64_t base = A.patch_off + A.patch_cnt[b];
  for (int i = tid; i < A.n_rec; i += 256) {
    if (!A.rr_mask[(size_t)b * A.n_rec + i]) continue;
    const int k0 = A.rr_start[i], n = A.rr_outdeg[i];
    for (int q = 0; q < n; ++q) {
      const int64_t pos = base + pre_[i] + q;
      A.e_src[pos] = rec0 + i; A.e_dst[pos] = rec0 + A.rr_dst[k0 + q]; A.e_aux[pos] = k0 + q;
    }
  }
}

hipError_t launch_disco_patch(const PatchArgs& a, hipStream_t s) {
// ... 495 lines not shown
```

disco_diffdock_amd/csrc/model.h:

```cpp
#pragma once
#include <stdio.h>
#include <stdlib.h>
#include <thread>

#include "ddk_internal.h"

namespace ddk {

constexpr int SIG = 32;
constexpr int DE = 32;
constexpr int MAX_LIG = 256;
constexpr int MAX_REC = 8192;
constexpr int LIG_CAP = 33;
constexpr int BOND_CAP = 32;
constexpr int LIG_DIMS[16] = {119, 4, 12, 12, 8, 10, 6, 6, 2, 8, 2, 2, 2, 2, 2, 2};
constexpr int REC_DIM = 38;

enum InfoSlot : int {
  I_GO = 5,
  I_CNT = 10,
  I_FB = 18,
  I_E = 24,
  I_OVF = 25,
  I_MISMATCH = 31,
  I_SEG = 27,
  I_SHARED = 26,
  I_TAB = 32,
  I_EXEC = 80,
  I_HEAD = 96,
  I_TABX = 104,
  I_PATCH = 114,
  I_FBX = 115,
  INFO_INTS = 128
};
enum GroupTable : int { TAB_ALL = 0, TAB_C = 1, TAB_B = 2, TAB_A = 3, TAB_SHARED = 4, N_TAB = 5 };
constexpr int CNT_STRIDE = 6;

struct StepParams {
  float lig_node_sig[NS], rec_node_sig[NS];
  float lig_edge_sigb[NS], rec_edge_sigb[NS], cross_edge_sigb[NS], center_edge_sigb[NS];
  float tr_sigb[NS], rot_sigb[NS];
  float tr_sigma, rot_sigma, tor_sigma;
  float so3_norm;
  float torus_norm_sqrt;
  float cross_cutoff;
};

struct EdgeMlpDev {
  const float* w1d;
  const float* w1b;
  const float* w2;
  const float* b2;
  const float* w1l;
  const float* unc;
  float coeff;
  float step;
  const float* offset;
  const float* w1d_t = nullptr;
  const float* w2_t = nullptr;
};

struct ModelDev {
  EdgeMlpDev lig_edge, rec_edge, cross_edge, center_edge, final_edge;
  const float* final_edge_b1;
  const float *lig_w_lat, *rec_w_lat;
  const float *lig_node_unc, *rec_node_unc;
  int latent_dim;
  const float *fc_w0, *fc_b0, *fc_w4, *fc_b4;
  float fc_bn_scale[4];
  const float *tr_w0n, *tr_w3, *rot_w0n, *rot_w3;
  float tr_b3, rot_b3;
  const float *tb_w0, *tb_b0, *tb_w4, *tb_b4;
  const float *tb_bn_scale, *tb_bn_mean, *tb_bn_bias;
  const float *tf_w0, *tf_w3;
  const float *rec_table, *rec_w_emb, *rec_w_lm_t, *rec_b;
};

constexpr int AR_H = 128;
constexpr int AR_NS_MAX = 24;
struct ArMlpDev { const float *w0, *b0, *w4, *b4, *w8; float b8; };
struct ArArgs {
  const float* x;
  ArMlpDev s, r;
  int ar_ns, H;
  int n_lig_total, n_rec_total, n_lig, n_rec;
  float* logits;
};
struct ArDecodeArgs {
  const float* logits;
  const float* uniforms;
  float temperature;
  int n_lig, n_rec, idx, latent_dim;
  float* lig_latent;
  float* rec_latent;
  int32_t* choices;
};
hipError_t launch_ar_logits(const ArArgs& A, hipStream_t s);
hipError_t launch_ar_decode(const ArDecodeArgs& A, int B, hipStream_t s);

struct ModelHost {
  std::vector<float> lig_tables;
  std::vector<int> lig_table_off;
  std::vector<float> lig_w_emb, lig_w_sig, lig_b;
  std::vector<float> rec_table, rec_w_emb, rec_w_esm, rec_w_sig, rec_b;
  std::vector<float> le_w1s, le_b1, re_w1s, re_b1, ce_w1s, ce_b1, cen_w1s, cen_b1;
  std::vector<float> re_w1d;
  std::vector<float> tr_w0s, tr_b0, rot_w0s, rot_b0;
  float rec_coeff = 0.f;
  std::vector<float> rec_offset;
  bool ready = false;
};

struct ConfPredictorDev {
  float *w0 = nullptr, *s0 = nullptr, *t0 = nullptr, *w4 = nullptr, *s4 = nullptr, *t4 = nullptr, *w8 = nullptr, *b8 = nullptr;
  int n_out = 1;
};
int conf_predictor_load(ddk_ctx* ctx, ConfPredictorDev& P);
hipError_t launch_conf_head(const ConfPredictorDev& P, const float* x, int B, int n_lig, float* out, const int32_t* ovf, hipStream_t s);

struct Model {
  ModelDev dev;
  ModelHost host;
  bool confidence_mode = false;
  ConfPredictorDev pred;
  bool has_ar = false;
  ArMlpDev ar_s, ar_r;
  int ar_ns = 0, ar_H = 0;
};


struct GraphArgs {
  const float* lig_pos;
  const float* rec_pos;
  const int32_t* bond_src;
  const int32_t* bond_dst;
  const int32_t* rr_src;
  const int32_t* rr_dst;
  const int32_t* rr_outdeg;
  int B, n_lig, n_rec, M, E_rr;
  float lig_r2;
  float cross_cutoff;
  const int32_t* rr_start;
  int32_t* counts;
  int32_t* offs;
  int32_t* info;
  uint8_t* levels;
  int prune = 0;
  int shared_rr = 0;
  int32_t* e_src;
  int32_t* e_dst;
  int32_t* e_aux;
  int32_t* deg;
  int rec_node_base = -1;
  int64_t patch_off = -1;
  int64_t edge_cap = 0;
  int cross_mirror = 0;
};

int det_ranges_count(int kind, int B);
hipError_t launch_det_ranges(const GraphArgs& G, int kind, int len_uniform, int32_t* out, hipStream_t s);

struct PatchArgs {
  const float* rec_latent;
  const int32_t* rr_start;
  const int32_t* rr_outdeg;
  const int32_t* rr_dst;
  int B, n_lig, n_rec, E_rr, latent_dim;
  int64_t patch_off;
  uint8_t* rr_mask;
  int32_t* patch_cnt;
  int32_t* info;
  int32_t *e_src, *e_dst, *e_aux;
};
hipError_t launch_disco_patch(const PatchArgs& a, hipStream_t s);

struct EdgeFeatArgs {
  const float* lig_pos;
  const float* rec_pos;
  const float* bond_attr;
  const float* rr_pre1;
  const float* rr_sh;
  const int32_t* e_src;
  const int32_t* e_dst;
  const int32_t* e_aux;
  const int32_t* info;
  float* e_emb;
  float* e_sh;
  EdgeMlpDev lig, rec, cross;
  StepParams sp;
  int n_lig_total;
  int rec_node_base = -1;
  int n_rec;
  int n_shared = 0;
  int cross_mirror = 0;
  int g2_live_only = 0;
  int64_t patch_off = -1;
  const float* lig_latent;
  const float* rec_latent;
  float unconditional;
  int latent_dim;
};

struct HeadArgs {
  const float* lig_pos;
  const float* x;
  ModelDev md;
  StepParams sp;
  int B, n_lig, R;
  int scale_by_sigma;
  const int32_t* rot_u;
  const int32_t* rot_v;
  float lig_r2;
  float* tr_out;
  float* rot_out;
  float* tor_out;
  int32_t *h_src, *h_dst, *h_deg, *h_info;
  float *h_attr, *h_sh, *h_sum;
  int32_t* prof_out = nullptr;
  const int32_t* exec_info = nullptr;
  int deterministic;
};

struct Se3Args {
  const float* pos;
  const float* tr;
  const float* rot;
  const float* tor;
  const float* noise;
  float sc[3], nc[3];
  const int32_t* rot_u;
  const int32_t* rot_v;
// ... 73 lines not shown
  int n_lig, n_rot;
  const float *pos0, *target;
  const uint8_t* atom_mask;
  const int32_t* rot_bonds;
  const uint8_t* mask_rotate;
};
struct MatchSearch { int popsize, maxiter, polish_iters, n_islands; float tol; uint64_t seed, stream_id; };
int64_t match_workspace_bytes(int n_lig, int n_rot, int popsize, int n_islands);
hipError_t launch_conformer_rmsd(const MatchProblem& P, int M, const float* torsions, float* rmsd_out, int32_t* status_out, hipStream_t s);
hipError_t launch_conformer_match(const MatchProblem& P, const MatchSearch& O, float* torsions_out, float* pos_out, float* rmsd_out, int32_t* count_out,
                                  void* workspace, hipStream_t s);

hipError_t launch_rng_noise(uint64_t seed, uint64_t stream_id, int sample0, int B, int step0, int steps, int n_cols, int n_active, float* out, hipStream_t s);
hipError_t launch_rng_initial(uint64_t seed, uint64_t stream_id, int sample0, int B, int n_rot, float tr_sigma, int purpose_rot, float* tor_out, float* rot_out,
                              float* tr_out, hipStream_t s);
hipError_t launch_rng_uniform(uint64_t seed, uint64_t stream_id, int sample0, int B, int decoding_idx, float* out, hipStream_t s);

constexpr int NOISE_BATCH_MAX_GRAPHS = 65536;
constexpr int NOISE_BATCH_MAX_ROWS = 4096;
constexpr int NOISE_BATCH_MAX_ROT = 1024;
struct ConformerBatchArgs {
  const float* pos;
  const int32_t *node_ptr, *tor_ptr, *mask_ptr;
  const int32_t* rot_bonds;
  const uint8_t* mask_rotate;
  const float *tr, *rot, *tor;
  int G, N, T, mask_bytes;
  float* pos_out;
  int32_t* status_out;
};
hipError_t launch_modify_conformer_batch(const ConformerBatchArgs& A, hipStream_t s);
struct RandPosBatchArgs {
  const float* pos;
  const int32_t *node_ptr, *tor_ptr, *mask_ptr;
  const int32_t* rot_bonds;
  const uint8_t* mask_rotate;
  const uint64_t* stream_id;
  const int32_t* sample;
  uint32_t seed_lo, seed_hi;
  float tr_sigma;
  int G, N, T, mask_bytes;
  float* pos_out;
  int32_t* status_out;
};
hipError_t launch_randomize_batch(const RandPosBatchArgs& A, hipStream_t s);

int conf_model_finalize(ddk_ctx* ctx);
void conf_complex_free(ddk_complex* cx);
void conf_model_destroy(ddk_ctx* ctx);
struct ConfComplex;

hipError_t launch_graph(const GraphArgs& G, int64_t edge_cap, hipStream_t s);
GraphArgs graph_args(const ddk_ctx* ctx, const ddk_complex* cx, int B, const float* lig_pos, float cross_cutoff);
int graph_cross_mirror_fits(int n_lig, int n_rec);
hipError_t launch_edge_features(const EdgeFeatArgs& A, int64_t edge_cap, hipStream_t s);
hipError_t launch_edge_features_node(const EdgeFeatArgs& A, int64_t edge_cap, const NodePreArgs& P, const NodeEmbedArgs& E, hipStream_t s);
struct NodeEmbedArgs {
  const float* lig_static; const float* rec_static; StepParams sp; int B, n_lig, n_rec; float* x;
  const float *lig_latent, *rec_latent, *lig_w_lat, *rec_w_lat, *lig_unc, *rec_unc; float unconditional; int latent_dim;
};
hipError_t launch_node_embed(const NodeEmbedArgs& a, hipStream_t s);
struct RecStaticArgs { const float* rec_x; int n_rec, feat_dim, lm; const float *rec_table, *w_emb, *w_lm_t, *b; float* out; };
hipError_t launch_complex_static(const RecStaticArgs& R, const int32_t* rr_src, const int32_t* rr_dst, const float* rec_pos, int E, const EdgeMlpDev& m,
                                 float* pre1, hipStream_t s);
hipError_t launch_zero_fill(void* p, size_t bytes, hipStream_t s);
hipError_t launch_heads_pre(const HeadArgs& A, bool torsion, hipStream_t s);
hipError_t launch_heads_post(const HeadArgs& A, bool torsion, hipStream_t s);
hipError_t launch_se3(const Se3Args& A, hipStream_t s, const HeadArgs* post = nullptr);
hipError_t launch_cfg_combine(float* score, const float* uncond, float weight, int64_t n, hipStream_t s);

}

struct ddk_complex {
  int n_lig = 0, n_rec = 0, M = 0, R = 0, E_rr = 0, max_batch = 0;
  int32_t *bond_src = nullptr, *bond_dst = nullptr, *rot_u = nullptr, *rot_v = nullptr, *rot_bond = nullptr;
  float* bond_attr = nullptr;
  uint8_t* mask_rotate = nullptr;
  float *rec_pos = nullptr, *lig_node_static = nullptr, *rec_node_static = nullptr;
  int32_t *rr_src = nullptr, *rr_dst = nullptr, *rr_outdeg = nullptr, *rr_start = nullptr;
  float *rr_pre1 = nullptr, *rr_sh = nullptr;
  int64_t edge_cap = 0;
  int32_t *e_src = nullptr, *e_dst = nullptr, *e_aux = nullptr, *deg = nullptr, *counts = nullptr, *offs = nullptr, *info = nullptr;
  uint8_t* levels = nullptr;
  float *e_emb = nullptr, *e_sh = nullptr, *xa = nullptr, *xb = nullptr, *sum = nullptr;
  float* scores = nullptr;
  const float *lig_latent = nullptr, *rec_latent = nullptr;
  float unconditional = 0.0f;
  int64_t patch_off = -1;
  uint8_t* rr_mask = nullptr;
  int32_t* patch_cnt = nullptr;
  bool latent_dirty = true;
  int patch_B = 0;
  float cfg_weight = 0.0f, cfg_start = 1.0f, cfg_end = 0.0f;
  float *zero_lat = nullptr, *scores2 = nullptr;
  float* part = nullptr;
  int32_t* det_rng = nullptr;
  float* sum_rr0 = nullptr;
  int32_t *h_src = nullptr, *h_dst = nullptr, *h_deg = nullptr;
  float *h_attr = nullptr, *h_sh = nullptr, *h_sum = nullptr;
  float* pre = nullptr;
  float* x_last = nullptr;
  int last_B = 0;
  bool sum_clean = false;
  bool keep_rec = false, last_full = false;
  ddk::ConfComplex* conf = nullptr;
  ddk_ctx* owner = nullptr;
  struct Chunk { void* p; size_t cap; };
  std::vector<Chunk> allocs;
  char* chunk = nullptr;
  size_t chunk_cap = 0, chunk_off = 0, reserve_hint = 0;
  bool oom = false;
  int stage_idx = -1;
  size_t stage_off = 0;
  struct CopyRec { void* dst; size_t off, bytes; };
  std::vector<CopyRec> pending;
  hipEvent_t ready = nullptr;
  bool ready_pending = false;
  hipStream_t last_stream = nullptr;
  std::vector<hipStream_t> streams;
  bool used = false;
  struct Canary { char* tail; size_t bytes; };
  std::vector<Canary> canaries;
  std::vector<int32_t> h_rr;
  std::vector<float> h_rec_pos;
};

#define GET(var, name, ...) const HostTensor* var = find_w(ctx, name, {__VA_ARGS__}); if (!var) return DDK_ERR_INVALID
#define CK(x, what) do { hipError_t ck_e = (x); if (ck_e != hipSuccess) return hip_fail(ctx, ck_e, what); } while (0)

namespace ddk {
const HostTensor* find_w(ddk_ctx* ctx, const std::string& name, std::initializer_list<int64_t> shape);
std::vector<float> cols(const HostTensor* t, int c0, int c1);
std::vector<float> transpose_rm(const std::vector<float>& w, int rows, int cols_);

template <typename F>
inline void host_parallel_for(int n, F&& body) {
  unsigned nt = std::thread::hardware_concurrency();
  nt = nt < 1 ? 1 : (nt > 8 ? 8 : nt);
  if (n < 512 || nt == 1) {
    for (int i = 0; i < n; ++i) body(i);
    return;
  }
  std::vector<std::thread> th;
  const int per = (n + (int)nt - 1) / (int)nt;
  for (unsigned t = 0; t < nt; ++t) {
    const int lo = (int)t * per, hi = lo + per < n ? lo + per : n;
    if (lo >= hi) break;
    th.emplace_back([lo, hi, &body]() { for (int i = lo; i < hi; ++i) body(i); });
  }
  for (auto& x : th) x.join();
}


void* cx_new_chunk(ddk_complex* cx, size_t cap);
int cx_stage_begin(ddk_ctx* ctx, ddk_complex* cx, size_t bytes);
bool cx_put(ddk_complex* cx, void* dst, const void* src, size_t bytes);
int cx_stage_flush(ddk_ctx* ctx, ddk_complex* cx);
hipError_t cx_wait_ready(ddk_complex* cx, hipStream_t s);
inline void cx_reserve(ddk_complex* cx, size_t bytes) { cx->reserve_hint = bytes; }
inline bool cx_canary_on() { static const bool on = getenv("DDK_CANARY") != nullptr; return on; }
inline void* cx_alloc(ddk_complex* cx, size_t bytes) {
  const size_t need = (((bytes ? bytes : 4) + 255) & ~(size_t)255) + (cx_canary_on() ? 4096 : 0);
  if (!cx->chunk || cx->chunk_off + need > cx->chunk_cap) {
    size_t cap = need > cx->reserve_hint ? need : cx->reserve_hint;
    if (cap < ((size_t)1 << 20)) cap = (size_t)1 << 20;
    void* p = cx_new_chunk(cx, cap);
// ... 25 lines not shown
```

disco_diffdock_amd/csrc/model.hip:

```cpp
#include <math.h>
#include <string.h>

#include <algorithm>
#include <thread>

#include "k_philox.h"
#include "model.h"

namespace ddk {

std::vector<float> cols(const HostTensor* t, int c0, int c1) {
  const int rows = (int)t->shape[0], nc = (int)t->shape[1];
  std::vector<float> o((size_t)rows * (c1 - c0));
  for (int r = 0; r < rows; ++r)
    for (int c = c0; c < c1; ++c) o[(size_t)r * (c1 - c0) + (c - c0)] = t->data[(size_t)r * nc + c];
  return o;
}

static bool smearing(ddk_ctx* ctx, const char* name, float stop, EdgeMlpDev& m, std::vector<float>* host_off, float* host_coeff) {
  std::vector<float> off(DE);
  auto it = ctx->weights.find(std::string(name) + "_distance_expansion.offset");
  if (it != ctx->weights.end() && it->second.data.size() == (size_t)DE) off = it->second.data;
  else for (int k = 0; k < DE; ++k) off[k] = stop * (float)k / (float)(DE - 1);
  const double d = (double)(off[1] - off[0]);
// ... 322 lines not shown
  cx->allocs.push_back({p, cap});
  cx->chunk_cap = cap;
  return p;
}

int cx_stage_begin(ddk_ctx* ctx, ddk_complex* cx, size_t bytes) {
  bytes = (bytes + 4095) & ~(size_t)4095;
  int idx = -1;
  for (int i = 0; i < (int)ctx->stage_pool.size(); ++i) {
    auto& b = ctx->stage_pool[i];
    if (b.in_flight && hipEventQuery(b.done) == hipSuccess) b.in_flight = false;
    if (!b.in_flight && b.cap >= bytes && (idx < 0 || b.cap < ctx->stage_pool[idx].cap)) idx = i;
  }
  if (idx < 0) {
    ddk_ctx::StageBuf b;
    b.cap = bytes < ((size_t)8 << 20) ? ((size_t)8 << 20) : bytes;
    if (hipHostMalloc((void**)&b.p, b.cap) != hipSuccess) return fail(ctx, DDK_ERR_NOMEM, "hipHostMalloc failed (staging buffer)");
    if (hipEventCreateWithFlags(&b.done, hipEventDisableTiming) != hipSuccess) return fail(ctx, DDK_ERR_HIP, "event create failed");
    ctx->stage_pool.push_back(b);
    idx = (int)ctx->stage_pool.size() - 1;
  }
  ctx->stage_pool[idx].in_flight = true;
  cx->stage_idx = idx; cx->stage_off = 0; cx->pending.clear();
  return DDK_OK;
}

bool cx_put(ddk_complex* cx, void* dst, const void* src, size_t bytes) {
  if (!dst || !bytes) return dst != nullptr;
  ddk_ctx* ctx = cx->owner;
  if (cx->stage_idx >= 0) {
    auto& b = ctx->stage_pool[cx->stage_idx];
    const size_t off = (cx->stage_off + 255) & ~(size_t)255;
    if (off + bytes <= b.cap) {
      memcpy(b.p + off, src, bytes);
      cx->stage_off = off + bytes;
      if (!cx->pending.empty()) {
        auto& l = cx->pending.back();
        const size_t gap = off - l.off;
        if ((char*)l.dst + gap == (char*)dst && gap >= l.bytes && gap - l.bytes < 256) { l.bytes = gap + bytes; return true; }
      }
      cx->pending.push_back({dst, off, bytes});
      return true;
    }
  }
  if (hipMemcpyAsync(dst, src, bytes, hipMemcpyHostToDevice, ctx->up_stream) != hipSuccess) return false;
  return hipStreamSynchronize(ctx->up_stream) == hipSuccess;
}

int cx_stage_flush(ddk_ctx* ctx, ddk_complex* cx) {
  hipError_t e = hipSuccess;
  if (cx->stage_idx >= 0) {
    auto& b = ctx->stage_pool[cx->stage_idx];
    for (const auto& r : cx->pending)
      if (e == hipSuccess) e = hipMemcpyAsync(r.dst, b.p + r.off, r.bytes, hipMemcpyHostToDevice, ctx->up_stream);
    if (e == hipSuccess) e = hipEventRecord(b.done, ctx->up_stream);
    cx->pending.clear();
    cx->stage_idx = -1;
  }
  if (e == hipSuccess && !cx->ready) e = hipEventCreateWithFlags(&cx->ready, hipEventDisableTiming);
  if (e == hipSuccess) e = hipEventRecord(cx->ready, ctx->up_stream);
  if (e != hipSuccess) return hip_fail(ctx, e, "complex upload");
  cx->ready_pending = true;
  return DDK_OK;
}

hipError_t cx_wait_ready(ddk_complex* cx, hipStream_t s) {
  cx->last_stream = s; cx->used = true;
  if (std::find(cx->streams.begin(), cx->streams.end(), s) == cx->streams.end()) cx->streams.push_back(s);
  if (!cx->ready_pending) return hipSuccess;
  if (hipEventQuery(cx->ready) == hipSuccess) { cx->ready_pending = false; return hipSuccess; }
  return hipStreamWaitEvent(s, cx->ready, 0);
}

GraphArgs graph_args(const ddk_ctx* ctx, const ddk_complex* cx, int B, const float* lig_pos, float cross_cutoff) {
  GraphArgs G;
  G.lig_pos = lig_pos; G.rec_pos = cx->rec_pos; G.bond_src = cx->bond_src; G.bond_dst = cx->bond_dst;
  G.rr_src = cx->rr_src; G.rr_dst = cx->rr_dst; G.rr_outdeg = cx->rr_outdeg; G.rr_start = cx->rr_start;
  G.B = B; G.n_lig = cx->n_lig; G.n_rec = cx->n_rec; G.M = cx->M; G.E_rr = cx->E_rr;
  G.lig_r2 = ctx->cfg.lig_max_radius * ctx->cfg.lig_max_radius; G.cross_cutoff = cross_cutoff; G.counts = cx->counts; G.offs = cx->offs; G.info = cx->info; G.levels = cx->levels;
  return G;
}

static hipError_t build_graph(ddk_ctx* ctx, ddk_complex* cx, int B, const float* lig_pos, float cross_cutoff, bool prune, bool shared_rr,
                              hipStream_t s, int64_t patch_off = -1, int cross_mirror = 0) {
  GraphArgs G = graph_args(ctx, cx, B, lig_pos, cross_cutoff);
  G.cross_mirror = cross_mirror; G.prune = prune ? 1 : 0; G.shared_rr = shared_rr ? 1 : 0; G.patch_off = patch_off;
  G.e_src = cx->e_src; G.e_dst = cx->e_dst; G.e_aux = cx->e_aux; G.deg = cx->deg;
  return launch_graph(G, cx->edge_cap, s);
}

static int score_forward_impl(ddk_ctx* ctx, ddk_complex* cx, int B, const float* lig_pos, const StepParams& sp,
                              float* tr_out, float* rot_out, float* tor_out, hipStream_t s, HeadArgs* defer_post = nullptr) {
  const ddk_config& c = ctx->cfg;
  Model* M = (Model*)ctx->model;
  const int n_lig = cx->n_lig, n_rec = cx->n_rec;
  const int64_t N = (int64_t)B * (n_lig + n_rec);
  const bool patched = c.latent_dim > 0 && ctx->layer0_dedup && !c.deterministic && cx->patch_off >= 0 && cx->pre != nullptr &&
                       ctx->conv[0].wn != nullptr && c.num_conv_layers > 1;
  const bool dedup = ((c.latent_dim == 0 && ctx->layer0_dedup) || patched) && B > 1 && cx->E_rr > 0;
  if (c.latent_dim > 0 && (!cx->lig_latent || !cx->rec_latent))
    return fail(ctx, DDK_ERR_STATE, "latent-conditioned model: call ddk_set_latents before the forward");
  if (dedup && patched && (cx->latent_dirty || cx->patch_B != B)) {
    PatchArgs P;
    P.rec_latent = cx->rec_latent; P.rr_start = cx->rr_start; P.rr_outdeg = cx->rr_outdeg; P.rr_dst = cx->rr_dst;
    P.B = B; P.n_lig = n_lig; P.n_rec = n_rec; P.E_rr = cx->E_rr; P.latent_dim = c.latent_dim; P.patch_off = cx->patch_off;
    P.rr_mask = cx->rr_mask; P.patch_cnt = cx->patch_cnt; P.info = cx->info; P.e_src = cx->e_src; P.e_dst = cx->e_dst; P.e_aux = cx->e_aux;
    CK(launch_disco_patch(P, s), "layer-0 patch group");
    cx->latent_dirty = false; cx->patch_B = B;
  }
  const bool prune = ctx->prune && !cx->keep_rec && cx->E_rr > 0;
  const int mirror = graph_cross_mirror_fits(n_lig, n_rec);
  CK(build_graph(ctx, cx, B, lig_pos, sp.cross_cutoff, prune, dedup, s, (dedup && patched) ? cx->patch_off : -1, mirror), "graph build");
  EdgeFeatArgs F;
  F.cross_mirror = mirror;
  F.lig_pos = lig_pos; F.rec_pos = cx->rec_pos; F.bond_attr = cx->bond_attr; F.rr_pre1 = cx->rr_pre1; F.rr_sh = cx->rr_sh;
  F.e_src = cx->e_src; F.e_dst = cx->e_dst; F.e_aux = cx->e_aux; F.info = cx->info; F.e_emb = cx->e_emb; F.e_sh = cx->e_sh;
  F.lig = M->dev.lig_edge; F.rec = M->dev.rec_edge; F.cross = M->dev.cross_edge; F.sp = sp;
  F.n_lig_total = B * n_lig; F.n_rec = n_rec; F.n_shared = dedup ? cx->E_rr : 0;
  F.g2_live_only = (dedup && prune && c.num_conv_layers == 5) ? 1 : 0;
  F.patch_off = (dedup && patched) ? cx->patch_off : -1;
  F.latent_dim = c.latent_dim; F.lig_latent = cx->lig_latent; F.rec_latent = cx->rec_latent; F.unconditional = cx->unconditional;
  const int64_t cap_b = (int64_t)B * ((int64_t)cx->M + (int64_t)n_lig * LIG_CAP + 2LL * n_lig * n_rec + cx->E_rr) + cx->E_rr;
  const int64_t feat_cap = (cap_b < cx->edge_cap ? cap_b : cx->edge_cap) + (F.patch_off >= 0 ? (int64_t)B * cx->E_rr + 256 : 0);
  float* xin = cx->xa;
  float* xout = cx->xb;
  NodeEmbedArgs NE_;
  NE_.lig_static = cx->lig_node_static; NE_.rec_static = cx->rec_node_static; NE_.sp = sp; NE_.B = B; NE_.n_lig = n_lig; NE_.n_rec = n_rec;
  NE_.x = xin; NE_.lig_latent = cx->lig_latent; NE_.rec_latent = cx->rec_latent; NE_.lig_w_lat = M->dev.lig_w_lat; NE_.rec_w_lat = M->dev.rec_w_lat;
  NE_.lig_unc = M->dev.lig_node_unc; NE_.rec_unc = M->dev.rec_node_unc; NE_.unconditional = cx->unconditional; NE_.latent_dim = c.latent_dim;
  const bool split = ctx->conv[0].wn != nullptr && cx->pre != nullptr;
  const bool recv_only = split && ctx->conv[0].sender_in_gemm1;
  const int role_mask = recv_only ? 0x3 : 0xF;
  if (split) {
    NodePreArgs PA = {};
    PA.x_out = xin; PA.n_lig_total = B * n_lig; PA.n_rec_total = B * n_rec; PA.n_rec = n_rec;
    PA.wn = ctx->conv[0].wn; PA.bnp = ctx->conv[0].bnp; PA.pre = cx->pre; PA.n_slots = 1; PA.lig_roles = role_mask; PA.rec_roles = role_mask;
    CK(launch_edge_features_node(F, feat_cap, PA, NE_, s), "edge features + node embed + node_pre");
  } else {
    CK(launch_edge_features(F, feat_cap, s), "edge features");
    CK(launch_node_embed(NE_, s), "node embed");
  }
  if (!cx->sum_clean) {
    CK(hipMemsetAsync(cx->sum, 0, (size_t)cx->max_batch * (n_lig + n_rec) * XW * sizeof(float) * (c.deterministic ? 2 : 1), s), "memset sum");
    CK(hipMemsetAsync(cx->sum_rr0, 0, (size_t)n_rec * XW * sizeof(float), s), "memset sum_rr0");
  }
  cx->sum_clean = false;
  bool rr0_dirty = false;
  const int NL = c.num_conv_layers;
  int32_t* prof_slot = nullptr;
  if (ctx->prof && ctx->prof_slots + 1 <= ctx->prof_cap) prof_slot = ctx->prof_edges + (size_t)PROF_INTS * ctx->prof_slots;
  for (int l = 0; l < NL; ++l) {
    const ConvLayerDev& L = ctx->conv[l];
    ConvLaunch a;
    a.x = xin; a.src = cx->e_src; a.dst = cx->e_dst; a.edge_attr = cx->e_emb; a.sh = cx->e_sh; a.sum = cx->sum;
    a.tile_info = cx->info; a.counter = cx->info + I_CNT + (l % 8); a.gather = 1;
    a.pre = split ? cx->pre : nullptr;
    const bool lig_only = (l == NL - 1 && !cx->keep_rec);
    const bool shared0 = dedup && l == 0;
    int tab = TAB_ALL;
    if (shared0) tab = TAB_SHARED;
    else if (prune && l == NL - 2) tab = TAB_A;
    else if (prune && l == NL - 3) tab = TAB_B;
    else if (prune && l == NL - 4) tab = TAB_C;
    a.gbeg = cx->info + I_TAB + 8 * tab; a.gend = a.gbeg + 4;
    a.n_groups = 4; a.n_active = lig_only ? 2 : 4; a.n_slots = 1; a.slots = 0;
    if (shared0 && patched) {
      a.gbeg = cx->info + I_TABX; a.gend = a.gbeg + 5; a.n_groups = 5; a.n_active = 5; a.wmap = 0x23210ull;
    }
    if (c.deterministic) {
      a.n_slots = 2; a.slots = (0u) | (1u << 2) | (0u << 4) | (1u << 6);
      a.part = cx->part; a.edge_bound = cap_b;
      const int kind = lig_only ? 0 : (shared0 ? 5 : (tab == TAB_A ? 1 : (tab == TAB_B ? 2 : (tab == TAB_C ? 3 : 4))));
      GraphArgs Gd = {};
      Gd.counts = cx->counts; Gd.B = B; Gd.M = cx->M; Gd.E_rr = cx->E_rr;
      CK(launch_det_ranges(Gd, kind, 0, cx->det_rng, s), "deterministic ranges");
      a.det_rng = cx->det_rng; a.det_nr = det_ranges_count(kind, B);
    }
    if (shared0) {
      rr0_dirty = true;
      a.sum_g2 = cx->sum_rr0; a.g2_node_off = B * n_lig;
    }
    if (l >= 8) CK(hipMemsetAsync(cx->info + I_CNT + (l % 8), 0, sizeof(int32_t), s), "counter reset");
    ddk_ctx::ProfRec pr;
    if (prof_slot) {
      CK(hipEventCreate(&pr.a), "event"); CK(hipEventCreate(&pr.b), "event");
      pr.layer = l; pr.slot = ctx->prof_slots; pr.tab = tab; pr.lig_only = lig_only; pr.r01_skipped = shared0 ? (patched ? -1 : (int64_t)(B - 1) * cx->E_rr) : 0;
      CK(hipEventRecord(pr.a, s), "event record");
    }
    if (ctx->conv_trace != nullptr && ctx->conv_trace_layer == l) { a.trace = ctx->conv_trace; a.trace_coarse = ctx->conv_trace_coarse; }
    CK(launch_conv_fused(L, a, ctx->n_cu, s), "conv_fused");
    if (prof_slot) {
      CK(hipEventRecord(pr.b, s), "event record");
      ctx->prof_recs.push_back(pr);
    }
    const bool clear_rr0 = rr0_dirty && !shared0;
    if (split && l + 1 < NL) {
      NodePreArgs PA = {};
      PA.sum = cx->sum; PA.deg = cx->deg; PA.x_in = xin; PA.bn_mean = L.bn_mean; PA.bn_scale = L.bn_scale; PA.bn_bias = L.bn_bias;
      PA.dout = L.dout; PA.x_out = xout; PA.sum_rr0 = shared0 ? cx->sum_rr0 : nullptr; PA.n_lig_total = B * n_lig; PA.n_rec_total = B * n_rec;
      PA.rr0_mask = (shared0 && patched) ? cx->rr_mask : nullptr;
      PA.n_rec = n_rec; PA.zero_extra = clear_rr0 ? cx->sum_rr0 : nullptr; PA.n_extra = clear_rr0 ? (int64_t)n_rec * XW : 0;
      PA.wn = ctx->conv[l + 1].wn; PA.bnp = ctx->conv[l + 1].bnp; PA.pre = cx->pre; PA.n_slots = c.deterministic ? 2 : 1;
      const bool next_lig_only = (l + 1 == NL - 1) && !cx->keep_rec;
      PA.lig_roles = (next_lig_only ? 0x7 : 0xF) & role_mask; PA.rec_roles = (next_lig_only ? 0x4 : 0xF) & role_mask;
      PA.levels = prune ? cx->levels : nullptr; PA.max_level = l == NL - 2 ? 0 : (l == NL - 3 ? 1 : (l == NL - 4 ? 2 : 3));
      CK(launch_node_finalize_pre(PA, true, s), "node_finalize_pre");
    } else
    CK(launch_node_finalize(cx->sum, cx->deg, xin, L.bn_mean, L.bn_scale, L.bn_bias, lig_only ? (int64_t)B * n_lig : N, L.dout, XW, xout, s,
                            shared0 ? cx->sum_rr0 : nullptr, (int64_t)B * n_lig, n_rec, 1, clear_rr0 ? cx->sum_rr0 : nullptr,
                            clear_rr0 ? (int64_t)n_rec * XW : 0, c.deterministic ? 2 : 1, (shared0 && patched) ? cx->rr_mask : nullptr), "node_finalize");
    if (clear_rr0) rr0_dirty = false;
    float* t = xin; xin = xout; xout = t;
  }
  cx->x_last = xin;
  cx->last_B = B;
  cx->last_full = cx->keep_rec;
  cx->sum_clean = !rr0_dirty;
  if (M->confidence_mode) return DDK_OK;
  const bool torsion = !c.no_torsion && tor_out != nullptr && cx->R > 0;
  HeadArgs Hd;
  Hd.lig_pos = lig_pos; Hd.x = xin; Hd.md = M->dev; Hd.sp = sp; Hd.B = B; Hd.n_lig = n_lig; Hd.R = cx->R;
  Hd.scale_by_sigma = c.scale_by_sigma; Hd.rot_u = cx->rot_u; Hd.rot_v = cx->rot_v; Hd.lig_r2 = c.lig_max_radius * c.lig_max_radius;
  Hd.tr_out = tr_out; Hd.rot_out = rot_out; Hd.tor_out = tor_out;
  Hd.h_src = cx->h_src; Hd.h_dst = cx->h_dst; Hd.h_deg = cx->h_deg; Hd.h_info = cx->info + I_HEAD; Hd.h_attr = cx->h_attr; Hd.h_sh = cx->h_sh;
  Hd.h_sum = cx->h_sum; Hd.deterministic = c.deterministic;
  if (prof_slot) {
    Hd.prof_out = prof_slot; Hd.exec_info = cx->info + I_EXEC;
    ctx->prof_slots += 1;
  }
  CK(launch_heads_pre(Hd, torsion, s), "heads_pre");
  int32_t* head_rng = nullptr;
  if (c.deterministic) {
    head_rng = cx->det_rng + (4 * (7 * (size_t)cx->max_batch + 1) + 8);
    GraphArgs Gd = {};
    Gd.B = B;
    CK(launch_det_ranges(Gd, 6, n_lig, head_rng, s), "deterministic ranges (head)");
  }
  if (torsion) {
// ... 670 lines not shown
  if (on && !ctx->prof_edges) {
    ctx->prof_cap = 32768;
    if (hipHostMalloc((void**)&ctx->prof_edges, (size_t)ctx->prof_cap * PROF_INTS * sizeof(int32_t)) != hipSuccess)
      return fail(ctx, DDK_ERR_NOMEM, "hipHostMalloc failed");
  }
  ctx->prof = on != 0;
  return DDK_OK;
}

int ddk_profile_read(ddk_ctx* ctx, double* out, int32_t n) {
  if (!ctx || !out) return DDK_ERR_INVALID;
  const int L = ctx->cfg.num_conv_layers;
  if (n < 5 * L) return fail(ctx, DDK_ERR_INVALID, "profile buffer too small");
  for (int i = 0; i < 5 * L; ++i) out[i] = 0.0;
  hipError_t e = hipDeviceSynchronize();
  if (e != hipSuccess) return hip_fail(ctx, e, "profile sync");
  for (auto& r : ctx->prof_recs) {
    float ms = 0.f;
    e = hipEventElapsedTime(&ms, r.a, r.b);
    if (e != hipSuccess) return hip_fail(ctx, e, "hipEventElapsedTime");
    const int32_t* pe = ctx->prof_edges + (size_t)PROF_INTS * r.slot;
    const double E = pe[0], E01 = pe[1];
    out[5 * r.layer] += ms;
    out[5 * r.layer + 1] += 1.0;
    out[5 * r.layer + 2] += r.lig_only ? E01 : (double)pe[2 + r.tab];
    out[5 * r.layer + 3] += r.lig_only ? E01 : (r.r01_skipped < 0 ? (double)pe[2 + r.tab] : E - (double)r.r01_skipped);
    out[5 * r.layer + 4] += E;
  }
  return DDK_OK;
}

int ddk_profile_read_forwards(ddk_ctx* ctx, double* out, int32_t max_forwards) {
  if (!ctx || !out || max_forwards < 0) return DDK_ERR_INVALID;
  hipError_t e = hipDeviceSynchronize();
  if (e != hipSuccess) return hip_fail(ctx, e, "profile sync");
  const int nf = ctx->prof_slots < max_forwards ? ctx->prof_slots : max_forwards;
  for (int i = 0; i < 4 * nf; ++i) out[i] = 0.0;
  for (auto& r : ctx->prof_recs) {
    if (r.slot >= nf) continue;
    float ms = 0.f;
    e = hipEventElapsedTime(&ms, r.a, r.b);
    if (e != hipSuccess) return hip_fail(ctx, e, "hipEventElapsedTime");
    const int32_t* pe = ctx->prof_edges + (size_t)PROF_INTS * r.slot;
    const double E = pe[0], E01 = pe[1];
    out[4 * r.slot] += ms;
    out[4 * r.slot + 1] += r.lig_only ? E01 : (double)pe[2 + r.tab];
    out[4 * r.slot + 2] += r.lig_only ? E01 : (r.r01_skipped < 0 ? (double)pe[2 + r.tab] : E - (double)r.r01_skipped);
    out[4 * r.slot + 3] = (double)pe[7];
  }
  return ctx->prof_slots;
}

int ddk_debug_conv_trace(ddk_ctx* ctx, int32_t layer, uint32_t* trace) {
  if (!ctx) return DDK_ERR_INVALID;
  ctx->conv_trace = trace; ctx->conv_trace_layer = layer % 100; ctx->conv_trace_coarse = layer / 100;
  return DDK_OK;
}

int ddk_debug_set_conv_workgroups(ddk_ctx* ctx, int32_t n) {
  if (!ctx || n < 1 || n > 1024) return DDK_ERR_INVALID;
  ctx->n_cu = n;
  return DDK_OK;
}

int ddk_debug_pool_stats(ddk_ctx* ctx, int64_t* out) {
  if (!ctx || !out) return DDK_ERR_INVALID;
  out[0] = ctx->pool_mallocs; out[1] = ctx->pool_reuses; out[2] = ctx->pool_frees; out[3] = (int64_t)ctx->chunk_pool_bytes;
  out[4] = (int64_t)ctx->chunk_pool.size(); out[5] = ctx->pool_bytes_out; out[6] = ctx->pool_bytes_out_peak; out[7] = ctx->dev_bytes;
  return DDK_OK;
}

int ddk_debug_set_alloc_limit(ddk_ctx* ctx, int64_t bytes) {
  if (!ctx || bytes < 0) return DDK_ERR_INVALID;
  ctx->alloc_limit = bytes;
  return DDK_OK;
}

int ddk_debug_set_layer0_dedup(ddk_ctx* ctx, int32_t on) {
  if (!ctx) return DDK_ERR_INVALID;
  ctx->layer0_dedup = on != 0;
  return DDK_OK;
}

int ddk_debug_read_patch(ddk_ctx* ctx, ddk_complex* cx, int32_t B, int32_t* counts, uint8_t* mask) {
  if (!ctx || !cx || !counts || !mask) return DDK_ERR_INVALID;
  if (cx->patch_off < 0 || B < 1 || B > cx->max_batch) return fail(ctx, DDK_ERR_STATE, "no patch group on this complex (latent-conditioned models only)");
  hipError_t e = hipDeviceSynchronize();
  if (e == hipSuccess) e = hipMemcpy(counts, cx->patch_cnt, (size_t)(B + 1) * sizeof(int32_t), hipMemcpyDeviceToHost);
  if (e == hipSuccess) e = hipMemcpy(mask, cx->rr_mask, (size_t)B * cx->n_rec, hipMemcpyDeviceToHost);
  return e == hipSuccess ? DDK_OK : hip_fail(ctx, e, "ddk_debug_read_patch");
}

int ddk_debug_kabsch(ddk_ctx* ctx, int32_t nb, int32_t n, const float* A, const float* B, float* R_out, float* t_out, void* stream) {
  if (!ctx || ctx->host_only) return DDK_ERR_STATE;
  if (nb < 1 || n < 1 || n > MAX_LIG || !A || !B || !R_out || !t_out) return fail(ctx, DDK_ERR_INVALID, "ddk_debug_kabsch: bad argument");
  hipError_t e = launch_debug_kabsch(A, B, nb, n, R_out, t_out, (hipStream_t)stream);
  return e == hipSuccess ? DDK_OK : hip_fail(ctx, e, "debug kabsch");
}

int ddk_debug_axis_angle(ddk_ctx* ctx, int32_t n, const float* aa, float* R_out, void* stream) {
  if (!ctx || ctx->host_only) return DDK_ERR_STATE;
  if (n < 1 || !aa || !R_out) return fail(ctx, DDK_ERR_INVALID, "ddk_debug_axis_angle: bad argument");
  hipError_t e = launch_debug_axis_angle(aa, n, R_out, (hipStream_t)stream);
  return e == hipSuccess ? DDK_OK : hip_fail(ctx, e, "debug axis angle");
}

int ddk_debug_read_edges(ddk_ctx* ctx, ddk_complex* cx, int64_t first, int64_t n, int32_t* src, int32_t* dst, float* emb, float* sh, int32_t* deg,
                         int64_t n_nodes) {
  if (!ctx || !cx) return DDK_ERR_INVALID;
  const int64_t e_alloc = cx->edge_cap + (cx->patch_off >= 0 ? (int64_t)cx->max_batch * cx->E_rr : 0);
  if (first < 0 || n < 0 || first + n > e_alloc || n_nodes < 0 || n_nodes > (int64_t)cx->max_batch * (cx->n_lig + cx->n_rec))
    return fail(ctx, DDK_ERR_INVALID, "ddk_debug_read_edges: range outside the complex' edge / node arrays");
  hipError_t e = hipDeviceSynchronize();
  if (e == hipSuccess && src && n) e = hipMemcpy(src, cx->e_src + first, n * 4, hipMemcpyDeviceToHost);
  if (e == hipSuccess && dst && n) e = hipMemcpy(dst, cx->e_dst + first, n * 4, hipMemcpyDeviceToHost);
  if (e == hipSuccess && emb && n) e = hipMemcpy(emb, cx->e_emb + first * NS, n * NS * 4, hipMemcpyDeviceToHost);
  if (e == hipSuccess && sh && n) e = hipMemcpy(sh, cx->e_sh + first * 4, n * 16, hipMemcpyDeviceToHost);
  if (e == hipSuccess && deg && n_nodes) e = hipMemcpy(deg, cx->deg, n_nodes * 4, hipMemcpyDeviceToHost);
  return e == hipSuccess ? DDK_OK : hip_fail(ctx, e, "ddk_debug_read_edges");
}

int ddk_debug_cross_mirror(ddk_ctx* ctx, ddk_complex* cx) {
  if (!ctx || !cx) return DDK_ERR_INVALID;
  return graph_cross_mirror_fits(cx->n_lig, cx->n_rec) ? 1 : 0;
}

}
```

disco_diffdock_amd/runtime.py:

```python
import collections
import ctypes as C
import os
import warnings
from types import SimpleNamespace

import numpy as np
import torch

from . import _lib

_DATA = os.path.join(os.path.dirname(os.path.abspath(__file__)), 'data')

DEFAULTS = dict(ns=24, nv=6, num_conv_layers=5, sigma_embed_dim=32, distance_embed_dim=32, cross_distance_embed_dim=32,
                lig_max_radius=5.0, rec_max_radius=30.0, cross_max_distance=80.0, center_max_distance=30.0,
                dynamic_max_cross=1, embedding_scale=1000.0, scale_by_sigma=1, no_torsion=0, batch_norm=1,
                latent_dim=0, latent_vocab=0, latent_droprate=0.0, lm_embedding_dim=1280,
                tr_sigma_min=0.1, tr_sigma_max=19.0, rot_sigma_min=0.03, rot_sigma_max=1.55,
                tor_sigma_min=0.03, tor_sigma_max=3.14, device=0, all_atoms=0, num_confidence_outputs=1, confidence_no_batchnorm=0,
                conv_kernel=0, deterministic=0, confidence_mode=0)

CONF_GROUPS = ('ll', 'lr', 'la', 'aa', 'al', 'ar', 'rr', 'rl', 'ra')
CONF_STATUS_INTS, CONF_OVERFLOW_WORD = 20, 19


# ... 218 lines not shown
        self._match_ws = {}

    def _check(self, rc, what):
        if rc != 0:
            raise RuntimeError(f'{what}: {self.L.ddk_last_error(self.h).decode()} (rc={rc})')

    def close(self):
        if getattr(self, 'h', None):
            self.L.ddk_destroy(self.h)
            self.h = None

    def __del__(self):
        try:
            self.close()
        except Exception:
            pass

    def load_state_dict(self, state_dict, prefix='', finalize=True):
        for k, v in state_dict.items():
            if not torch.is_tensor(v) or not v.is_floating_point():
                continue
            a = np.ascontiguousarray(v.detach().cpu().float().numpy())
            shape = (C.c_int64 * max(a.ndim, 1))(*a.shape)
            self._check(self.L.ddk_load_weights(self.h, (prefix + k).encode(), a.ctypes.data_as(C.c_void_p), shape, a.ndim),
                        f'ddk_load_weights({k})')
        if finalize:
            self.finalize()

    def finalize(self):
        if not self._tables_set:
            self.set_tables(np.load(os.path.join(_DATA, 'so3_exp_score_norms.npy')),
                            np.load(os.path.join(_DATA, 'torus_score_norm_seed0.npy')))
        self._check(self.L.ddk_finalize_weights(self.h), 'ddk_finalize_weights')

    def set_tables(self, so3, torus):
        so3 = np.ascontiguousarray(so3, dtype=np.float64)
        torus = np.ascontiguousarray(torus, dtype=np.float64)
        self._check(self.L.ddk_set_score_norm_tables(self.h, so3.ctypes.data_as(C.c_void_p), len(so3),
                                                     torus.ctypes.data_as(C.c_void_p), len(torus)), 'ddk_set_score_norm_tables')
        self._tables_set = True
        self.score_norm_tables = (so3, torus)

    def export(self, what, dtype=np.float32):
        n = self.L.ddk_debug_export(self.h, what.encode(), None, 0)
        if n < 0:
            raise RuntimeError(f'ddk_debug_export({what}): {self.L.ddk_last_error(self.h).decode()}')
        buf = np.zeros(n, dtype=dtype)
        self.L.ddk_debug_export(self.h, what.encode(), buf.ctypes.data_as(C.c_void_p), n)
        return buf

    def profile_enable(self, on=True):
        self._check(self.L.ddk_profile_enable(self.h, int(on)), 'ddk_profile_enable')

    def profile_read(self):
        n = 5 * self.cfg.num_conv_layers
        buf = (C.c_double * n)()
        self._check(self.L.ddk_profile_read(self.h, buf, n), 'ddk_profile_read')
        a = np.array(list(buf)).reshape(-1, 5)
        return [dict(ms=float(r[0]), launches=int(r[1]), edges=int(r[2]), edges_unpruned=int(r[3]), edges_reference=int(r[4])) for r in a]

    def profile_read_forwards(self, max_forwards=32768):
        buf = (C.c_double * (4 * max_forwards))()
        n = self.L.ddk_profile_read_forwards(self.h, buf, max_forwards)
        if n < 0:
            raise RuntimeError(f'ddk_profile_read_forwards: {self.L.ddk_last_error(self.h).decode()}')
        if n >= max_forwards:
            raise RuntimeError(f'ddk_profile_read_forwards: {n} forwards recorded, the profile buffer holds {max_forwards}: later launches were not timed')
        return np.array(buf[:4 * min(n, max_forwards)]).reshape(-1, 4)

    def set_pruning(self, on=True):
        self._check(self.L.ddk_set_receptive_field_pruning(self.h, int(bool(on))), 'ddk_set_receptive_field_pruning')

    def pool_stats(self):
        buf = (C.c_int64 * 8)()
        self._check(self.L.ddk_debug_pool_stats(self.h, buf), 'ddk_debug_pool_stats')
        keys = ('hipMalloc_calls', 'reuses', 'hipFree_calls', 'bytes_parked', 'chunks_parked', 'bytes_owned', 'bytes_owned_peak', 'device_bytes_held')
        return dict(zip(keys, [int(v) for v in buf[:8]]))

    def debug_set_alloc_limit(self, nbytes=0):
        self._check(self.L.ddk_debug_set_alloc_limit(self.h, int(nbytes)), 'ddk_debug_set_alloc_limit')

    def debug_set_layer0_dedup(self, on=True):
        self._check(self.L.ddk_debug_set_layer0_dedup(self.h, int(bool(on))), 'ddk_debug_set_layer0_dedup')

    def tp_forward(self, layer, x_dst, sh, w, dout):
        x_dst, sh, w = x_dst.contiguous().float(), sh.contiguous().float(), w.contiguous().float()
        E = x_dst.shape[0]
        out = torch.empty((E, dout), dtype=torch.float32, device=x_dst.device)
        self._check(self.L.ddk_tp_forward(self.h, layer, _ptr(x_dst), _ptr(sh), _ptr(w), E, _ptr(out), _stream()), 'ddk_tp_forward')
        return out

    def tp_backward(self, layer, x_dst, sh, w, grad_out, need=(True, True, True)):
        need_x, need_sh, need_w = (bool(n) for n in need)
        if not (need_x or need_sh or need_w):
            raise RuntimeError('ddk: tp_backward needs at least one gradient to compute')
        if w is None and (need_x or need_sh):
            raise RuntimeError('ddk: tp_backward needs w for grad_x and grad_sh')
        x_dst, sh, grad_out = (_need_cuda(t).contiguous().float() for t in (x_dst, sh, grad_out))
        E = x_dst.shape[0]
        if need_x or need_sh:
            w = _need_cuda(w).contiguous().float()
            if w.dim() != 2 or w.shape[0] != E:
                raise RuntimeError('ddk: tp_backward takes w [E, W]; got ' + str(tuple(w.shape)))
            W = w.shape[1]
        else:
            w, W = None, self.tp_weight_numel(layer)
        if sh.shape != (E, 4) or grad_out.dim() != 2 or grad_out.shape[0] != E:
            raise RuntimeError('ddk: tp_backward takes sh [E, 4] and grad_out [E, Dout]')
        new = lambda cols: torch.empty((E, cols), dtype=torch.float32, device=x_dst.device)
        gx, gsh, gw = new(x_dst.shape[1]) if need_x else None, new(4) if need_sh else None, new(W) if need_w else None
        if E == 0:
            return gx, gsh, gw
        self._check(self.L.ddk_tp_backward(self.h, layer, _ptr(x_dst), _ptr(sh), _ptr(w), _ptr(grad_out), E, _ptr(gx), _ptr(gsh), _ptr(gw), _stream()),
                    'ddk_tp_backward')
        return gx, gsh, gw

    def _rtp_operands(self, layer, x_dst, sh, h, group_offsets, w2, b2, E=None):
        x_dst, sh, h = (_need_cuda(t).contiguous().float() for t in (x_dst, sh, h))
        offs = [int(o) for o in group_offsets]
        G, E, W = len(offs) - 1, x_dst.shape[0] if E is None else E, self.tp_weight_numel(layer)
        if not 1 <= G <= 4:
            raise RuntimeError(f'ddk: the radial tensor product takes 1..4 edge groups; got {G}')
        if sh.shape != (E, 4) or h.shape != (E, 72):
            raise RuntimeError('ddk: the radial tensor product takes sh [E, 4] and h [E, 72]')
        if w2 is not None:
            w2 = _need_cuda(w2).contiguous().float()
            if w2.shape != (G, W, 72):
                raise RuntimeError(f'ddk: the radial tensor product takes w2 [G, W, 72] = {(G, W, 72)}; got {tuple(w2.shape)}')
        if b2 is not None:
            b2 = _need_cuda(b2).contiguous().float()
            if b2.shape != (G, W):
                raise RuntimeError(f'ddk: the radial tensor product takes b2 [G, W] = {(G, W)}; got {tuple(b2.shape)}')
        return x_dst, sh, h, (C.c_int64 * (G + 1))(*offs), G, w2, b2, E, W

    def rtp_forward(self, layer, x_dst, sh, h, group_offsets, w2, b2, dout):
        x_dst, sh, h, offs, G, w2, b2, E, W = self._rtp_operands(layer, x_dst, sh, h, group_offsets, w2, b2)
        if w2 is None or b2 is None:
            raise RuntimeError('ddk: rtp_forward needs w2 and b2')
        out = torch.empty((E, dout), dtype=torch.float32, device=x_dst.device)
        self._check(self.L.ddk_rtp_forward(self.h, layer, _ptr(x_dst), _ptr(sh), _ptr(h), offs, G, _ptr(w2), _ptr(b2), E, _ptr(out), _stream()), 'ddk_rtp_forward')
        return out

    def rtp_backward(self, layer, x_dst, sh, h, group_offsets, w2, b2, grad_out, need=(True, True, True, True, True)):
        need = _need(need, 'rtp_backward')
        if w2 is None and any(need[:3]):
            raise RuntimeError('ddk: rtp_backward needs w2 for grad_x, grad_sh and grad_h')
        if b2 is None and any(need[:2]):
            raise RuntimeError('ddk: rtp_backward needs b2 for grad_x and grad_sh')
        x_dst, sh, h, offs, G, w2, b2, E, W = self._rtp_operands(layer, x_dst, sh, h, group_offsets, w2, b2)
        grad_out = _need_cuda(grad_out).contiguous().float()
        if grad_out.dim() != 2 or grad_out.shape[0] != E:
            raise RuntimeError('ddk: rtp_backward takes grad_out [E, Dout]')
        outs, live = _outputs(need, ((E, x_dst.shape[1]), (E, 4), (E, 72), (G, W, 72), (G, W)), x_dst.device)
        if not live:
            return tuple(outs)
        ws = None
        if need[3] or need[4]:
            ws = _workspace(self.L.ddk_rtp_backward_workspace(layer, E, G), f'rtp_backward: no workspace for layer {layer}, E = {E}, {G} groups', x_dst.device)
        self._check(self.L.ddk_rtp_backward(self.h, layer, _ptr(x_dst), _ptr(sh), _ptr(h), offs, G, _ptr(w2), _ptr(b2), _ptr(grad_out), E,
                                            *[_ptr(o) for o in outs], _ptr(ws), _stream()), 'ddk_rtp_backward')
        return tuple(outs)

    @staticmethod
    def conv_graph(edge_src, edge_dst, n_in, n_out):
        src, dst = torch.as_tensor(edge_src).reshape(-1), torch.as_tensor(edge_dst).reshape(-1)
        n_in, n_out, E = int(n_in), int(n_out), src.shape[0]
# ... 1209 lines not shown
```

include/ddk_debug.h:

```cpp
#ifndef DDK_DEBUG_H
#define DDK_DEBUG_H

#include "ddk.h"

#ifdef __cplusplus
extern "C" {
#endif

int64_t ddk_debug_export(ddk_ctx* ctx, const char* what, void* buf, int64_t cap_words);

int ddk_debug_read_edges(ddk_ctx* ctx, ddk_complex* cx, int64_t first, int64_t n, int32_t* src, int32_t* dst, float* emb, float* sh, int32_t* deg,
                         int64_t n_nodes);

int ddk_debug_cross_mirror(ddk_ctx* ctx, ddk_complex* cx);

int ddk_debug_conf_counts(ddk_ctx* ctx, ddk_complex* cx, int32_t* out);
int ddk_debug_conf_table(ddk_ctx* ctx, ddk_complex* cx, int32_t which, int32_t* out);
int ddk_debug_conf_nodes(ddk_ctx* ctx, ddk_complex* cx, float* x, int32_t* deg, int64_t n);
int ddk_debug_conf_edges(ddk_ctx* ctx, ddk_complex* cx, int64_t first, int64_t n, int32_t* src, int32_t* dst, float* emb, float* sh,
                         int32_t* gt);

int ddk_debug_set_layer0_dedup(ddk_ctx* ctx, int32_t on);

int ddk_debug_pool_stats(ddk_ctx* ctx, int64_t* out);
int ddk_debug_set_alloc_limit(ddk_ctx* ctx, int64_t bytes);

int ddk_debug_set_conv_workgroups(ddk_ctx* ctx, int32_t n);
int ddk_debug_read_patch(ddk_ctx* ctx, ddk_complex* cx, int32_t B, int32_t* counts, uint8_t* mask);

int ddk_debug_kabsch(ddk_ctx* ctx, int32_t nb, int32_t n, const float* A, const float* B, float* R_out, float* t_out, void* stream);
int ddk_debug_axis_angle(ddk_ctx* ctx, int32_t n, const float* aa, float* R_out, void* stream);

int ddk_debug_conv_trace(ddk_ctx* ctx, int32_t layer, uint32_t* trace);

int ddk_debug_split3(ddk_ctx* ctx, const float* x, int64_t n, int32_t group, float* hi, float* mid, float* lo, float* scale, void* stream);

#ifdef __cplusplus
}
#endif
#endif
```

Measured before the change: 51.93.

## Share rec-rec edge feature rows across batch instead of materializing per-sample copies

When layer-0 dedup is on and the model has no latent conditioning, the graph builder stops writing per-sample edge embedding and spherical harmonic rows for receptor-receptor edges. Conv kernels instead redirect those edges to a single shared row block, using a static edge id stored in the aux array plus a base offset from the info table. This removes the edge-feature writes for B copies of the rec-rec edges and shrinks the feature buffer. In exchange, each edge does an extra indirect load in the conv kernels, and lanes 62/63 are repurposed to carry the base and offset. A debug toggle and a reconstruction path in the debug edge reader are added.

```diff
diff --git a/disco_diffdock_amd/_lib.py b/disco_diffdock_amd/_lib.py
--- a/disco_diffdock_amd/_lib.py
+++ b/disco_diffdock_amd/_lib.py
@@ -63,7 +63,7 @@
            'ddk_rng_perturbation_batch', 'ddk_rng_forward_times', 'ddk_modify_conformer_batch', 'ddk_randomize_position_batch', 'ddk_score_matching_loss_batch',
            'ddk_score_matching_loss_batch_backward']
 
-DEBUG_SYMBOLS = ['ddk_debug_export', 'ddk_debug_read_edges', 'ddk_debug_conf_counts', 'ddk_debug_conf_table', 'ddk_debug_conf_nodes', 'ddk_debug_conf_edges', 'ddk_debug_kabsch', 'ddk_debug_axis_angle', 'ddk_debug_set_layer0_dedup', 'ddk_debug_read_patch', 'ddk_debug_split3', 'ddk_debug_conv_trace', 'ddk_debug_pool_stats', 'ddk_debug_set_conv_workgroups', 'ddk_debug_set_alloc_limit', 'ddk_debug_cross_mirror']
+DEBUG_SYMBOLS = ['ddk_debug_export', 'ddk_debug_read_edges', 'ddk_debug_conf_counts', 'ddk_debug_conf_table', 'ddk_debug_conf_nodes', 'ddk_debug_conf_edges', 'ddk_debug_kabsch', 'ddk_debug_axis_angle', 'ddk_debug_set_layer0_dedup', 'ddk_debug_read_patch', 'ddk_debug_split3', 'ddk_debug_conv_trace', 'ddk_debug_pool_stats', 'ddk_debug_set_conv_workgroups', 'ddk_debug_set_alloc_limit', 'ddk_debug_cross_mirror', 'ddk_debug_set_edge_row_sharing']
 
 
 def lib():
@@ -197,6 +197,7 @@
     L.ddk_debug_kabsch.argtypes = [C.c_void_p, C.c_int32, C.c_int32, C.c_void_p, C.c_void_p, C.c_void_p, C.c_void_p, C.c_void_p]
     L.ddk_debug_axis_angle.argtypes = [C.c_void_p, C.c_int32, C.c_void_p, C.c_void_p, C.c_void_p]
     L.ddk_debug_set_layer0_dedup.argtypes = [C.c_void_p, C.c_int32]
+    L.ddk_debug_set_edge_row_sharing.argtypes = [C.c_void_p, C.c_int32]
     L.ddk_debug_read_patch.argtypes = [C.c_void_p, C.c_void_p, C.c_int32, C.c_void_p, C.c_void_p]
     L.ddk_debug_split3.argtypes = [C.c_void_p, C.c_void_p, C.c_int64, C.c_int32, C.c_void_p, C.c_void_p, C.c_void_p, C.c_void_p, C.c_void_p]
     L.ddk_debug_conv_trace.argtypes = [C.c_void_p, C.c_int32, C.c_void_p]
diff --git a/disco_diffdock_amd/csrc/conv_launch.hip b/disco_diffdock_amd/csrc/conv_launch.hip
--- a/disco_diffdock_amd/csrc/conv_launch.hip
+++ b/disco_diffdock_amd/csrc/conv_launch.hip
@@ -186,6 +186,7 @@
     }
   }
   if (key.det && key.gather && !key.split) return hipErrorInvalidValue;
+  if (key.gather && key.mode == 0 && (a.aux == nullptr || a.row_base == nullptr || a.aux - a.src != (int64_t)(int32_t)(a.aux - a.src))) return hipErrorInvalidValue;
   return hipSuccess;
 }
 
@@ -198,6 +199,8 @@
   k.n_cols = L.n_cols;
   for (int c = 0; c <= L.n_cols; ++c) k.col_start[c] = L.col_start[c];
   k.sum_g2 = a.sum_g2; k.g2_node_off = a.g2_node_off;
+  if (a.aux != nullptr) k.aux_off = (int)(a.aux - a.src);
+  k.row_base = a.row_base;
   k.n_groups = a.n_groups; k.n_active = a.n_active; k.n_slots = a.n_slots; k.slots = a.slots; k.wmap = a.wmap;
   if (a.gbeg) { k.gbeg = a.gbeg; k.gend = a.gend; }
   else { k.gbeg = a.tile_info + 5; k.gend = a.tile_info + 6; }
diff --git a/disco_diffdock_amd/csrc/ddk_internal.h b/disco_diffdock_amd/csrc/ddk_internal.h
--- a/disco_diffdock_amd/csrc/ddk_internal.h
+++ b/disco_diffdock_amd/csrc/ddk_internal.h
@@ -195,6 +195,7 @@
   bool prof = false;
   bool prune = true;
   uint32_t* conv_trace = nullptr; int conv_trace_layer = -1; int conv_trace_coarse = 0;
+  bool edge_row_sharing = true;
   bool layer0_dedup = true;
   struct ProfRec { hipEvent_t a, b; int layer; int slot; int tab = 0; int64_t r01_skipped = 0; bool lig_only = false; };
   std::vector<ProfRec> prof_recs;
@@ -229,6 +230,8 @@
   int gather;
   float* sum_g2 = nullptr;
   int g2_node_off = 0;
+  const int32_t* aux = nullptr;
+  const int32_t* row_base = nullptr;
   int mode = 0;
   int n_groups = 4, n_active = 4, n_slots = 1;
   uint32_t slots = 0;
diff --git a/disco_diffdock_amd/csrc/k_conv.hip b/disco_diffdock_amd/csrc/k_conv.hip
--- a/disco_diffdock_amd/csrc/k_conv.hip
+++ b/disco_diffdock_amd/csrc/k_conv.hip
@@ -52,6 +52,7 @@
   const int el = lane & 31;
   const int hh = lane >> 5;
   const bool g2_shared = A.sum_g2 != nullptr;
+  constexpr bool ROWS = GATHER && MODE == 0;
   int gb_v = 0, ge_v = 0;
   if (lane < A.n_active) {
     gb_v = A.gbeg[lane];
@@ -65,6 +66,7 @@
     if (lane >= d) pend_v += t;
   }
   const int pbeg_v = pend_v - nb_v;
+  if constexpr (ROWS) conv_rows_park(A, lane, gb_v);
   int bs4 = __builtin_amdgcn_readlane(pend_v, 15);
   if constexpr (DET) {
     if (A.det_nr > 0) bs4 = A.det_rng[A.det_nr];
@@ -114,6 +116,7 @@
     const bool valid = el < nvalid;
     const int e = nvalid > 0 ? e0 + min(el, nvalid - 1) : gend - 1;
     const int sn = A.src[e], dn = A.dst[e];
+    const int er = ROWS ? conv_edge_row(A, gb_v, g, e) : e;
 
     const int gw = (int)((A.wmap >> (4 * g)) & 15);
     const float* wrec = A.w2r + (size_t)gw * n_tiles * W2_TILE_FLOATS;
@@ -137,7 +140,7 @@
     if constexpr (SPLIT) {
       float bin[12];
       {
-        const float* pe = A.edge_attr + (size_t)e * NS + 12 * hh;
+        const float* pe = A.edge_attr + (size_t)er * NS + 12 * hh;
 #pragma unroll
         for (int j = 0; j < 3; ++j) {
           const float4 a = ld4(pe + 4 * j);
@@ -181,7 +184,7 @@
     {
       const float *pe, *pxs, *pxd;
       if (GATHER) {
-        pe = A.edge_attr + (size_t)e * NS + 12 * hh;
+        pe = A.edge_attr + (size_t)er * NS + 12 * hh;
         pxs = A.x + (size_t)sn * XW + 12 * hh;
         pxd = A.x + (size_t)dn * XW + 12 * hh;
       } else {
@@ -229,7 +232,7 @@
     }
     }
 
-    const float4 shv = ld4(A.sh + (size_t)e * 4);
+    const float4 shv = ld4(A.sh + (size_t)er * 4);
     const float s0 = shv.x, vx = shv.y, vy = shv.z, vz = shv.w;
     {
       const float* xr = A.x + (size_t)dn * XW;
diff --git a/disco_diffdock_amd/csrc/k_conv_common.h b/disco_diffdock_amd/csrc/k_conv_common.h
--- a/disco_diffdock_amd/csrc/k_conv_common.h
+++ b/disco_diffdock_amd/csrc/k_conv_common.h
@@ -34,7 +34,19 @@
   const int32_t* gend;
   const int32_t* det_rng = nullptr;
   int det_nr = 0;
+  int aux_off = 0;
+  const int32_t* row_base = nullptr;
 };
+constexpr int CONV_LANE_ROW_BASE = 63, CONV_LANE_AUX_OFF = 62;
+__device__ __forceinline__ void conv_rows_park(const ConvKArgs& A, int lane, int& gb_v) {
+  if (lane == CONV_LANE_ROW_BASE) gb_v = *A.row_base;
+  if (lane == CONV_LANE_AUX_OFF) gb_v = A.aux_off;
+}
+__device__ __forceinline__ int conv_edge_row(const ConvKArgs& A, int gb_v, int g, int e) {
+  const int base = __builtin_amdgcn_readlane(gb_v, CONV_LANE_ROW_BASE), off = __builtin_amdgcn_readlane(gb_v, CONV_LANE_AUX_OFF);
+  const int k = A.src[(int64_t)e + off];
+  return (g == 2 && base >= 0) ? base + k : e;
+}
 struct DetRange { int beg, end, g, bstart; };
 __device__ __forceinline__ DetRange det_find(const int32_t* rng, int nr, int blk) {
   int lo = 0, hi = nr;
diff --git a/disco_diffdock_amd/csrc/k_conv_x.hip b/disco_diffdock_amd/csrc/k_conv_x.hip
--- a/disco_diffdock_amd/csrc/k_conv_x.hip
+++ b/disco_diffdock_amd/csrc/k_conv_x.hip
@@ -262,6 +262,7 @@
   const int el = lane & 31;
   const int hh = lane >> 5;
   const bool g2_shared = A.sum_g2 != nullptr;
+  constexpr bool ROWS = GATHER && MODE == 0;
   int gb_v = 0, ge_v = 0;
   if (lane < A.n_active) {
     gb_v = A.gbeg[lane];
@@ -275,6 +276,7 @@
     if (lane >= d) pend_v += t;
   }
   const int pbeg_v = pend_v - nb_v;
+  if constexpr (ROWS) conv_rows_park(A, lane, gb_v);
   int bs4 = __builtin_amdgcn_readlane(pend_v, 15);
   if constexpr (DET) {
     if (A.det_nr > 0) bs4 = A.det_rng[A.det_nr];
@@ -339,6 +341,7 @@
     const bool valid = el < nvalid;
     const int e = nvalid > 0 ? e0 + min(el, nvalid - 1) : gend - 1;
     const int sn = A.src[e], dn = A.dst[e];
+    const int er = ROWS ? conv_edge_row(A, gb_v, g, e) : e;
 
     const int gw = (int)((A.wmap >> (4 * g)) & 15);
     const char* wrec = reinterpret_cast<const char*>(A.w2x) + (size_t)gw * n_tiles * X3_TILE_BYTES;
@@ -390,7 +393,7 @@
     float2 pv2[3 * NV / 2];
     const float* xr = A.x + (size_t)dn * XW;
     if constexpr (!SENDK) {
-      shv = ld4(A.sh + (size_t)e * 4);
+      shv = ld4(A.sh + (size_t)er * 4);
 #pragma unroll
       for (int j = 0; j < NS / 4; ++j) mainv[j] = ld4(xr + (hh ? OFF_C : 0) + 4 * j);
 #pragma unroll
@@ -414,7 +417,7 @@
         }
         float bin[24];
         {
-          const float* pe = A.edge_attr + (size_t)e * NS + 12 * hh;
+          const float* pe = A.edge_attr + (size_t)er * NS + 12 * hh;
 #pragma unroll
           for (int j = 0; j < 3; ++j) {
             const float4 a = ld4(pe + 4 * j);
@@ -423,7 +426,7 @@
 #pragma unroll
           for (int j = 0; j < 3; ++j) mainv[j] = ld4(xr + 12 * hh + 4 * j);
         }
-        shv = ld4(A.sh + (size_t)e * 4);
+        shv = ld4(A.sh + (size_t)er * 4);
 #pragma unroll
         for (int j = 0; j < 3; ++j) mainv[3 + j] = ld4(xr + OFF_C + 12 * hh + 4 * j);
 #pragma unroll
@@ -475,7 +478,7 @@
         }
         float bin[12];
         {
-          const float* pe = A.edge_attr + (size_t)e * NS + 12 * hh;
+          const float* pe = A.edge_attr + (size_t)er * NS + 12 * hh;
 #pragma unroll
           for (int j = 0; j < 3; ++j) {
             const float4 a = ld4(pe + 4 * j);
@@ -531,7 +534,7 @@
         {
           const float *pe, *pxs, *pxd;
           if (GATHER) {
-            pe = A.edge_attr + (size_t)e * NS + 12 * hh;
+            pe = A.edge_attr + (size_t)er * NS + 12 * hh;
             pxs = A.x + (size_t)sn * XW + 12 * hh;
             pxd = A.x + (size_t)dn * XW + 12 * hh;
           } else {
diff --git a/disco_diffdock_amd/csrc/k_graph.hip b/disco_diffdock_amd/csrc/k_graph.hip
--- a/disco_diffdock_amd/csrc/k_graph.hip
+++ b/disco_diffdock_amd/csrc/k_graph.hip
@@ -207,7 +207,8 @@
   int bs = 0;
   G.info[I_FB] = 0;
   for (int g = 0; g < 5; ++g) {
-    bs += (g == 3 && G.cross_mirror) ? 0 : ((g < 4 ? go[g + 1] - go[g] : n_shared) + 255) / 256;
+    const bool none = (g == 3 && G.cross_mirror) || (g == 2 && G.share_rows && G.shared_rr);
+    bs += none ? 0 : ((g < 4 ? go[g + 1] - go[g] : n_shared) + 255) / 256;
     G.info[I_FB + 1 + g] = bs;
   }
   for (int g = 0; g < 5; ++g) G.info[I_GO + g] = go[g];
@@ -216,6 +217,7 @@
   G.info[I_E] = go[4];
   G.info[I_OVF] = ((int64_t)go[4] + n_shared > G.edge_cap) ? 1 : 0;
   G.info[I_SHARED] = G.shared_rr ? go[4] : -1;
+  G.info[I_ROWS] = (G.share_rows && G.shared_rr && !G.info[I_OVF]) ? go[4] : -1;
   G.info[I_HEAD] = 0; G.info[I_HEAD + 1] = G.B * G.n_lig; G.info[I_HEAD + 2] = G.B * G.n_lig; G.info[I_HEAD + 3] = G.B * G.n_lig;
   G.info[I_HEAD + 4] = 0; G.info[I_HEAD + 5] = 0;
   G.info[I_EXEC] = go[4];
diff --git a/disco_diffdock_amd/csrc/model.h b/disco_diffdock_amd/csrc/model.h
--- a/disco_diffdock_amd/csrc/model.h
+++ b/disco_diffdock_amd/csrc/model.h
@@ -31,6 +31,7 @@
   I_TABX = 104,
   I_PATCH = 114,
   I_FBX = 115,
+  I_ROWS = 116,
   INFO_INTS = 128
 };
 enum GroupTable : int { TAB_ALL = 0, TAB_C = 1, TAB_B = 2, TAB_A = 3, TAB_SHARED = 4, N_TAB = 5 };
@@ -147,6 +148,7 @@
   uint8_t* levels;
   int prune = 0;
   int shared_rr = 0;
+  int share_rows = 0;
   int32_t* e_src;
   int32_t* e_dst;
   int32_t* e_aux;
@@ -386,6 +388,7 @@
   int64_t edge_cap = 0;
   int32_t *e_src = nullptr, *e_dst = nullptr, *e_aux = nullptr, *deg = nullptr, *counts = nullptr, *offs = nullptr, *info = nullptr;
   uint8_t* levels = nullptr;
+  bool rows_shared = false;
   float *e_emb = nullptr, *e_sh = nullptr, *xa = nullptr, *xb = nullptr, *sum = nullptr;
   float* scores = nullptr;
   const float *lig_latent = nullptr, *rec_latent = nullptr;
diff --git a/disco_diffdock_amd/csrc/model.hip b/disco_diffdock_amd/csrc/model.hip
--- a/disco_diffdock_amd/csrc/model.hip
+++ b/disco_diffdock_amd/csrc/model.hip
@@ -428,9 +428,9 @@
 }
 
 static hipError_t build_graph(ddk_ctx* ctx, ddk_complex* cx, int B, const float* lig_pos, float cross_cutoff, bool prune, bool shared_rr,
-                              hipStream_t s, int64_t patch_off = -1, int cross_mirror = 0) {
+                              hipStream_t s, int64_t patch_off = -1, int cross_mirror = 0, bool share_rows = false) {
   GraphArgs G = graph_args(ctx, cx, B, lig_pos, cross_cutoff);
-  G.cross_mirror = cross_mirror; G.prune = prune ? 1 : 0; G.shared_rr = shared_rr ? 1 : 0; G.patch_off = patch_off;
+  G.cross_mirror = cross_mirror; G.prune = prune ? 1 : 0; G.shared_rr = shared_rr ? 1 : 0; G.patch_off = patch_off; G.share_rows = (shared_rr && share_rows) ? 1 : 0;
   G.e_src = cx->e_src; G.e_dst = cx->e_dst; G.e_aux = cx->e_aux; G.deg = cx->deg;
   return launch_graph(G, cx->edge_cap, s);
 }
@@ -456,7 +456,9 @@
   }
   const bool prune = ctx->prune && !cx->keep_rec && cx->E_rr > 0;
   const int mirror = graph_cross_mirror_fits(n_lig, n_rec);
-  CK(build_graph(ctx, cx, B, lig_pos, sp.cross_cutoff, prune, dedup, s, (dedup && patched) ? cx->patch_off : -1, mirror), "graph build");
+  const bool share_rows = dedup && c.latent_dim == 0 && ctx->edge_row_sharing;
+  cx->rows_shared = share_rows;
+  CK(build_graph(ctx, cx, B, lig_pos, sp.cross_cutoff, prune, dedup, s, (dedup && patched) ? cx->patch_off : -1, mirror, share_rows), "graph build");
   EdgeFeatArgs F;
   F.cross_mirror = mirror;
   F.lig_pos = lig_pos; F.rec_pos = cx->rec_pos; F.bond_attr = cx->bond_attr; F.rr_pre1 = cx->rr_pre1; F.rr_sh = cx->rr_sh;
@@ -467,7 +469,8 @@
   F.patch_off = (dedup && patched) ? cx->patch_off : -1;
   F.latent_dim = c.latent_dim; F.lig_latent = cx->lig_latent; F.rec_latent = cx->rec_latent; F.unconditional = cx->unconditional;
   const int64_t cap_b = (int64_t)B * ((int64_t)cx->M + (int64_t)n_lig * LIG_CAP + 2LL * n_lig * n_rec + cx->E_rr) + cx->E_rr;
-  const int64_t feat_cap = (cap_b < cx->edge_cap ? cap_b : cx->edge_cap) + (F.patch_off >= 0 ? (int64_t)B * cx->E_rr + 256 : 0);
+  const int64_t feat_cap = (cap_b < cx->edge_cap ? cap_b : cx->edge_cap) + (F.patch_off >= 0 ? (int64_t)B * cx->E_rr + 256 : 0) -
+                           (share_rows ? (int64_t)B * cx->E_rr : 0);
   float* xin = cx->xa;
   float* xout = cx->xb;
   NodeEmbedArgs NE_;
@@ -500,6 +503,7 @@
     ConvLaunch a;
     a.x = xin; a.src = cx->e_src; a.dst = cx->e_dst; a.edge_attr = cx->e_emb; a.sh = cx->e_sh; a.sum = cx->sum;
     a.tile_info = cx->info; a.counter = cx->info + I_CNT + (l % 8); a.gather = 1;
+    a.aux = cx->e_aux; a.row_base = cx->info + I_ROWS;
     a.pre = split ? cx->pre : nullptr;
     const bool lig_only = (l == NL - 1 && !cx->keep_rec);
     const bool shared0 = dedup && l == 0;
@@ -1336,6 +1340,12 @@
   return DDK_OK;
 }
 
+int ddk_debug_set_edge_row_sharing(ddk_ctx* ctx, int32_t on) {
+  if (!ctx) return DDK_ERR_INVALID;
+  ctx->edge_row_sharing = on != 0;
+  return DDK_OK;
+}
+
 int ddk_debug_read_patch(ddk_ctx* ctx, ddk_complex* cx, int32_t B, int32_t* counts, uint8_t* mask) {
   if (!ctx || !cx || !counts || !mask) return DDK_ERR_INVALID;
   if (cx->patch_off < 0 || B < 1 || B > cx->max_batch) return fail(ctx, DDK_ERR_STATE, "no patch group on this complex (latent-conditioned models only)");
@@ -1371,6 +1381,24 @@
   if (e == hipSuccess && emb && n) e = hipMemcpy(emb, cx->e_emb + first * NS, n * NS * 4, hipMemcpyDeviceToHost);
   if (e == hipSuccess && sh && n) e = hipMemcpy(sh, cx->e_sh + first * 4, n * 16, hipMemcpyDeviceToHost);
   if (e == hipSuccess && deg && n_nodes) e = hipMemcpy(deg, cx->deg, n_nodes * 4, hipMemcpyDeviceToHost);
+  if (e == hipSuccess && cx->rows_shared && n && (emb || sh)) {
+    int32_t info[INFO_INTS];
+    e = hipMemcpy(info, cx->info, sizeof(info), hipMemcpyDeviceToHost);
+    const int64_t base = info[I_ROWS], lo = std::max<int64_t>(first, info[I_GO + 2]), hi = std::min<int64_t>(first + n, info[I_GO + 3]);
+    if (e == hipSuccess && base >= 0 && lo < hi) {
+      std::vector<int32_t> aux((size_t)(hi - lo));
+      std::vector<float> remb((size_t)cx->E_rr * NS), rsh((size_t)cx->E_rr * 4);
+      e = hipMemcpy(aux.data(), cx->e_aux + lo, (size_t)(hi - lo) * 4, hipMemcpyDeviceToHost);
+      if (e == hipSuccess) e = hipMemcpy(remb.data(), cx->e_emb + base * NS, remb.size() * 4, hipMemcpyDeviceToHost);
+      if (e == hipSuccess) e = hipMemcpy(rsh.data(), cx->e_sh + base * 4, rsh.size() * 4, hipMemcpyDeviceToHost);
+      for (int64_t q = lo; e == hipSuccess && q < hi; ++q) {
+        const int32_t k = aux[(size_t)(q - lo)];
+        if (k < 0 || k >= cx->E_rr) return fail(ctx, DDK_ERR_STATE, "ddk_debug_read_edges: a rec-rec edge without a static id");
+        if (emb) memcpy(emb + (q - first) * NS, remb.data() + (size_t)k * NS, NS * 4);
+        if (sh) memcpy(sh + (q - first) * 4, rsh.data() + (size_t)k * 4, 16);
+      }
+    }
+  }
   return e == hipSuccess ? DDK_OK : hip_fail(ctx, e, "ddk_debug_read_edges");
 }
 
diff --git a/disco_diffdock_amd/runtime.py b/disco_diffdock_amd/runtime.py
--- a/disco_diffdock_amd/runtime.py
+++ b/disco_diffdock_amd/runtime.py
@@ -324,6 +324,9 @@
 
     def debug_set_layer0_dedup(self, on=True):
         self._check(self.L.ddk_debug_set_layer0_dedup(self.h, int(bool(on))), 'ddk_debug_set_layer0_dedup')
+
+    def debug_set_edge_row_sharing(self, on=True):
+        self._check(self.L.ddk_debug_set_edge_row_sharing(self.h, int(bool(on))), 'ddk_debug_set_edge_row_sharing')
 
     def tp_forward(self, layer, x_dst, sh, w, dout):
         x_dst, sh, w = x_dst.contiguous().float(), sh.contiguous().float(), w.contiguous().float()
diff --git a/include/ddk_debug.h b/include/ddk_debug.h
--- a/include/ddk_debug.h
+++ b/include/ddk_debug.h
@@ -22,6 +22,8 @@
 
 int ddk_debug_set_layer0_dedup(ddk_ctx* ctx, int32_t on);
 
+int ddk_debug_set_edge_row_sharing(ddk_ctx* ctx, int32_t on);
+
 int ddk_debug_pool_stats(ddk_ctx* ctx, int64_t* out);
 int ddk_debug_set_alloc_limit(ddk_ctx* ctx, int64_t bytes);
 
```

New measurement: 52.08, median of 6. No clear change (+0.3%).
